# zhyever/PatchFusion

Hardware: AMD Instinct MI355X
Metric: patches/sec (DepthAnything-ViT-L PatchFusion, 4K image, P=16 tiles at N=1) (higher is better)
Workload: dtype f32; 1 GPU; Depth-Anything-vitl14 PatchFusion, 2160x3840 synthetic RGB, 4x4 regular tiling (cai_mode m1, 16 tiles), process_num=8, random-init weights (BASELINE.json configs[2] at N=1; 16 tiles per GPU); parallelism=single GPU

## Files before the change

include/pf_hip.h:

```cpp
#ifndef PF_HIP_H
#define PF_HIP_H
#include <stdint.h>

#ifdef __cplusplus
extern "C" {
#endif

#define PF_DTYPE_F32 0
#define PF_DTYPE_BF16 1

#define PF_ACT_NONE 0
#define PF_ACT_RELU 1
#define PF_ACT_GELU 2
#define PF_ACT_SOFTPLUS 3

const char* pf_last_error(void);
int pf_version(void);

typedef struct {
  const void* x; int x_ld; int B, H, W, Cin;
  const void* w; int w_rows; int Kpad;
  const float* bias; const float* scale;
  const void* res; int res_ld; const void* res2; int res2_ld;
  void* y; int y_ld; int OH, OW, Cout;
  int KH, KW, stride, pad;
  int act;
  int relu_in;
  int out_f32;
  int shuffle;
  int dtype;
  int korder;
  int batch;
  long x_bstride, w_bstride, y_bstride;
  const int* col_exp;
  const int* out_exp;
} pf_conv_params;
int pf_conv(const pf_conv_params* p, void* stream);
int pf_conv_timed(const pf_conv_params* p, int iters, float* ms, void* stream);

int pf_conv_winograd(const pf_conv_params* p, int m, const void* U, int u_rows, int u_kpad, void* V, void* M, void* stream);
int pf_conv_winograd_split3(const pf_conv_params* p, const void* U3, int u_rows, int u_kpad, void* V3, void* M, void* stream);
int pf_conv_winograd_split3_windowed(const pf_conv_params* p, const void* U3, int u_rows, int u_kpad, void* V3, void* M, long window, void* stream);
long pf_wino_f16x2_scratch_bytes(int cin, int u_rows);
int pf_conv_winograd_f16x2_supported(const pf_conv_params* p, int u_rows, int u_kpad, long window);
int pf_conv_winograd_f16x2_windowed(const pf_conv_params* p, const void* U, int u_rows, int u_kpad, void* V2, void* M, void* scratch, long window,
                                    void* stream);
int pf_gemm_f16x2_points(const pf_conv_params* p, const int* col_exp, int grid_cap, void* stream);
int pf_gemm_f16x2(const pf_conv_params* p, void* stream);

int pf_conv_winograd_fused_supported(const pf_conv_params* p);
int pf_conv_winograd_fused(const pf_conv_params* p, const void* up, int nnb, int gs, void* stream);
int pf_conv_winograd_fused_timed(const pf_conv_params* p, const void* up, int nnb, int gs, int iters, float* ms, void* stream);

int pf_gemm_split3(const pf_conv_params* p, void* stream);
int pf_conv1x1_split3(const pf_conv_params* p, const void* w3, int w3_rows, void* stream);
int pf_gemm_split3_ex(const pf_conv_params* p, int grid_cap, void* stream);
#define PF_S3_ROUTE_TILE64 0
#define PF_S3_ROUTE_TILE128 1
#define PF_S3_ROUTE_PERSIST128 2
#define PF_S3_ROUTE_PERSIST192 3
int pf_gemm_split3_route(const pf_conv_params* p, int cus);
int pf_gemm_split3_timed(const pf_conv_params* p, int iters, float* ms, void* stream);
int pf_gemm_bf16_pp(const pf_conv_params* p, void* stream);
int pf_layernorm_split3(const float* x, int x_ld, void* y3, int y_ld, long plane, int kmajor, const float* g, const float* b, float eps,
                        long rows, int D, void* stream);
int pf_layernorm_f16x2(const float* x, int x_ld, void* y2, const int* in_exp, const float* g, const float* b, float eps, long rows, int D,
                       void* stream);
int pf_vit_attention_qkv_split3(const void* qkv, void* out3, long plane, int kmajor, int B, int S, int Hh, void* stream);
int pf_vit_attention_split3(const void* qkv3, long plane_in, void* out3, long plane_out, int kmajor, int B, int S, int Hh, void* stream);
int pf_vit_attention_split3_v2(const void* qkv3, long plane_in, void* out3, long plane_out, int kmajor, int B, int S, int Hh, int queries_per_wave,
                               int schedule, void* stream);
int pf_vit_attention_split3_rpb(const void* qkv3, long plane_in, void* out3, long plane_out, int kmajor, int B, int S, int Hh, const float* tab,
                                int th, int tw, int queries_per_wave, void* stream);
int pf_split3(const float* x, int x_ld, void* y, int y_ld, long plane, long rows, int cols, void* stream);

int pf_patch_im2col(const float* img, int B, int H, int W, void* out, int ld, int dtype, void* stream);
int pf_patch_im2col_norm(const float* img, int B, int H, int W, int patch, const float* mean3, const float* std3, float* out, int ld, void* stream);
int pf_readout_concat(const float* x, int x_ld, int B, int S, int D, float* y, int y_ld, void* stream);
int pf_assemble_tokens(const void* emb, void* tokens, const float* cls, const float* pos, int B, int S, int D, int dtype,
                       void* stream);
int pf_layernorm(const void* x, int x_ld, void* y, int y_ld, const float* g, const float* b, float eps,
                 int batches, int in_rows_per_batch, int in_row_offset, int out_rows_per_batch, int D,
                 int dtype, void* stream);
int pf_qkv_split(const void* qkv, int B, int S, int Hh, void* q, void* k, void* vt, int Sp, float scale,
                 int dtype, void* stream);
int pf_vit_attention(const void* q, const void* k, const void* vt, void* out, int B, int S, int Sp, int Hh,
                     int dtype, void* stream);
int pf_vit_attention_qkv(const void* qkv, void* out, int B, int S, int Hh, int dtype, void* stream);

int pf_swin_ln_partition(const void* x, int x_ld, void* xw, const float* g, const float* b, float eps,
                         int B, int H, int W, int C, int shift, int dtype, void* stream);
int pf_swin_window_attention(const void* qkv, void* out, const float* bias_table, int B, int Hp, int Wp,
                             int C, int heads, int shift, int dtype, void* stream);
int pf_swin_unpartition_add(const void* proj, const void* shortcut, int s_ld, void* y, int y_ld, int B, int H,
                            int W, int C, int shift, int dtype, void* stream);
int pf_add_rowwise(void* x, int x_ld, const float* pos, int B, int T, int C, int dtype, void* stream);

int pf_resize_bilinear(const void* x, int x_ld, int B, int H, int W, int C, void* y, int y_ld, int OH, int OW,
                       const void* add, int add_ld, int in_f32, int out_f32, int dtype, void* stream);
int pf_resize_concat(const void* const* xs, const int* lds, const int* Hs, const int* Ws, const int* Cs, int nsrc, int B,
                     void* y, int y_ld, int OH, int OW, int dtype, void* stream);
int pf_crop_resize_planar(const float* img, int C, int H, int W, const int* boxes, int P, float* out, int oh, int ow,
                          void* stream);
int pf_roi_align(const void* feat, int f_ld, int Bf, int H, int W, int C, const float* rois, int K, void* y,
                 int y_ld, int oh, int ow, float spatial_scale, int in_f32, int out_f32, int dtype, void* stream);
int pf_maxpool2(const void* x, int x_ld, int B, int H, int W, int C, void* y, int y_ld, int dtype, void* stream);
int pf_copy_channels(const void* x, int x_ld, void* y, int y_ld, long npix, int C, int in_f32, int out_f32,
                     int dtype, void* stream);
int pf_pack_fusion_input(const float* cdepth, const float* fdepth, const float* crops, void* y, int B, int h, int w,
                         int dtype, void* stream);
int pf_nhwc_to_nchw_f32(const void* x, int x_ld, float* y, int B, int H, int W, int C, int in_f32, int dtype, void* stream);

int pf_attractor(const float* A, int a_ld, int n_attr, int a_stride, float a_eps, int attractor_exp, int kind_sum,
                 const float* b_prev, int hp, int wp, float* out, int B, int h, int w, int n_bins, void* stream);
int pf_seed_bin_centers(const float* x, int x_ld, float* out, long npix, int n_bins, float min_depth, float max_depth, int bounded,
                        int normalize, void* stream);
int pf_bounded_bin_centers(const float* b, float* out, long npix, int n_bins, float min_depth, float max_depth, void* stream);
int pf_logbinom_depth(const float* pt, int pt_ld, const float* centers, int hc, int wc, float* depth, int B, int h,
                      int w, int n_bins, float min_temp, float max_temp, void* stream);
int pf_bins_tail(const float* clb, int clb_ld, int rel_off, const float* emb, int he, int we, const float* w0f, const float* b0,
                 const float* w2, const float* b2, const float* centers, int hc, int wc, float* depth, int B, int H, int W, int nq,
                 float min_temp, float max_temp, void* stream);

int pf_stitch_init(float* pred, float* count, int MH, int MW, const float* depth, const float* mask, const int* yx,
                   int P, int ph, int pw, void* stream);
int pf_stitch_finish_init(float* avg, const float* pred, const float* count, long n, void* stream);
int pf_stitch_update(float* avg, float* count, int MH, int MW, const float* depth, int dh, int dw, const float* mask,
                     int y0, int x0, int ph, int pw, void* stream);
int pf_resize_nearest_f32(const float* x, int H, int W, float* y, int OH, int OW, void* stream);
int pf_resize_bilinear_f32(const float* x, int H, int W, float* y, int OH, int OW, void* stream);


int pf_u8_bicubic_to_f32(const uint8_t* src, int H, int W, int reverse_channels, float* dst, int OH, int OW, void* stream);

int pf_percentile_workspace_bytes(void);
int pf_percentiles_f32(const float* x, long n, float invalid_val, int use_invalid, const uint8_t* invalid_mask, double q0, double q1,
                       float* out2, void* workspace, void* stream);

int pf_colorize_f32(const float* depth, long n, const float* vmin_vmax, const uint8_t* lut_rgba, int N, float invalid_val,
                    int use_invalid, const uint8_t* invalid_mask, uint32_t background_rgba, uint8_t* out_rgba, void* stream);

int pf_depth_to_u16(const float* depth, long n, float scale, uint16_t* out, void* stream);

int pf_depth_metrics(const float* gt, int H, int W, const float* pred, int ph, int pw, const float* edges,
                     const uint8_t* additional_mask, float min_depth, float max_depth, int crop_y0, int crop_y1, int crop_x0, int crop_x1,
                     double* out13, void* stream);

int pf_silog_loss(const float* pred, const float* target, long n, float min_depth, float max_depth, float beta, double* ws3,
                  float* loss, void* stream);

#ifdef __cplusplus
}
#endif
#endif
```

patchfusion_amd/_lib.py:

```python
import ctypes as C
import os

import torch

_HERE = os.path.dirname(os.path.abspath(__file__))
LIB_PATH = os.environ.get("PF_LIB_PATH") or os.path.join(_HERE, "libpf_hip.so")

vp, ci, cf, cl = C.c_void_p, C.c_int, C.c_float, C.c_long


class ConvParams(C.Structure):
    _fields_ = [
        ("x", vp), ("x_ld", ci), ("B", ci), ("H", ci), ("W", ci), ("Cin", ci),
        ("w", vp), ("w_rows", ci), ("Kpad", ci),
        ("bias", vp), ("scale", vp),
        ("res", vp), ("res_ld", ci), ("res2", vp), ("res2_ld", ci),
        ("y", vp), ("y_ld", ci), ("OH", ci), ("OW", ci), ("Cout", ci),
        ("KH", ci), ("KW", ci), ("stride", ci), ("pad", ci),
        ("act", ci), ("relu_in", ci), ("out_f32", ci), ("shuffle", ci), ("dtype", ci), ("korder", ci),
        ("batch", ci), ("x_bstride", C.c_long), ("w_bstride", C.c_long), ("y_bstride", C.c_long),
        ("col_exp", vp), ("out_exp", vp),
    ]


SIGNATURES = {
    "pf_conv": [C.POINTER(ConvParams), vp],
    "pf_conv_timed": [C.POINTER(ConvParams), ci, C.POINTER(cf), vp],
    "pf_patch_im2col": [vp, ci, ci, ci, vp, ci, ci, vp],
    "pf_assemble_tokens": [vp, vp, vp, vp, ci, ci, ci, ci, vp],
    "pf_layernorm": [vp, ci, vp, ci, vp, vp, cf, ci, ci, ci, ci, ci, ci, vp],
    "pf_qkv_split": [vp, ci, ci, ci, vp, vp, vp, ci, cf, ci, vp],
    "pf_vit_attention": [vp, vp, vp, vp, ci, ci, ci, ci, ci, vp],
    "pf_vit_attention_qkv": [vp, vp, ci, ci, ci, ci, vp],
    "pf_swin_ln_partition": [vp, ci, vp, vp, vp, cf, ci, ci, ci, ci, ci, ci, vp],
    "pf_swin_window_attention": [vp, vp, vp, ci, ci, ci, ci, ci, ci, ci, vp],
    "pf_swin_unpartition_add": [vp, vp, ci, vp, ci, ci, ci, ci, ci, ci, ci, vp],
    "pf_add_rowwise": [vp, ci, vp, ci, ci, ci, ci, vp],
    "pf_resize_bilinear": [vp, ci, ci, ci, ci, ci, vp, ci, ci, ci, vp, ci, ci, ci, ci, vp],
    "pf_resize_concat": [C.POINTER(vp), C.POINTER(ci), C.POINTER(ci), C.POINTER(ci), C.POINTER(ci), ci, ci, vp, ci, ci, ci, ci, vp],
    "pf_crop_resize_planar": [vp, ci, ci, ci, vp, ci, vp, ci, ci, vp],
    "pf_roi_align": [vp, ci, ci, ci, ci, ci, vp, ci, vp, ci, ci, ci, cf, ci, ci, ci, vp],
    "pf_maxpool2": [vp, ci, ci, ci, ci, ci, vp, ci, ci, vp],
    "pf_copy_channels": [vp, ci, vp, ci, cl, ci, ci, ci, ci, vp],
    "pf_pack_fusion_input": [vp, vp, vp, vp, ci, ci, ci, ci, vp],
    "pf_nhwc_to_nchw_f32": [vp, ci, vp, ci, ci, ci, ci, ci, ci, vp],
    "pf_conv_winograd": [C.POINTER(ConvParams), ci, vp, ci, ci, vp, vp, vp],
    "pf_conv_winograd_split3": [C.POINTER(ConvParams), vp, ci, ci, vp, vp, vp],
    "pf_conv_winograd_split3_windowed": [C.POINTER(ConvParams), vp, ci, ci, vp, vp, C.c_long, vp],
    "pf_conv_winograd_f16x2_windowed": [C.POINTER(ConvParams), vp, ci, ci, vp, vp, vp, C.c_long, vp],
    "pf_gemm_f16x2_points": [C.POINTER(ConvParams), vp, ci, vp],
    "pf_gemm_f16x2": [C.POINTER(ConvParams), vp],
    "pf_gemm_split3": [C.POINTER(ConvParams), vp],
    "pf_gemm_split3_ex": [C.POINTER(ConvParams), ci, vp],
    "pf_conv1x1_split3": [C.POINTER(ConvParams), vp, ci, vp],
    "pf_gemm_split3_timed": [C.POINTER(ConvParams), ci, C.POINTER(cf), vp],
    "pf_gemm_bf16_pp": [C.POINTER(ConvParams), vp],
    "pf_split3": [vp, ci, vp, ci, cl, cl, ci, vp],
    "pf_layernorm_split3": [vp, ci, vp, ci, cl, ci, vp, vp, cf, cl, ci, vp],
    "pf_layernorm_f16x2": [vp, ci, vp, vp, vp, vp, cf, cl, ci, vp],
    "pf_vit_attention_qkv_split3": [vp, vp, cl, ci, ci, ci, ci, vp],
    "pf_vit_attention_split3": [vp, cl, vp, cl, ci, ci, ci, ci, vp],
    "pf_vit_attention_split3_v2": [vp, cl, vp, cl, ci, ci, ci, ci, ci, ci, vp],
    "pf_vit_attention_split3_rpb": [vp, cl, vp, cl, ci, ci, ci, ci, vp, ci, ci, ci, vp],
    "pf_patch_im2col_norm": [vp, ci, ci, ci, ci, vp, vp, vp, ci, vp],
    "pf_readout_concat": [vp, ci, ci, ci, ci, vp, ci, vp],
    "pf_conv_winograd_fused": [C.POINTER(ConvParams), vp, ci, ci, vp],
    "pf_conv_winograd_fused_timed": [C.POINTER(ConvParams), vp, ci, ci, ci, C.POINTER(cf), vp],
    "pf_attractor": [vp, ci, ci, ci, cf, ci, ci, vp, ci, ci, vp, ci, ci, ci, ci, vp],
    "pf_seed_bin_centers": [vp, ci, vp, cl, ci, cf, cf, ci, ci, vp],
    "pf_bounded_bin_centers": [vp, vp, cl, ci, cf, cf, vp],
    "pf_logbinom_depth": [vp, ci, vp, ci, ci, vp, ci, ci, ci, ci, cf, cf, vp],
    "pf_bins_tail": [vp, ci, ci, vp, ci, ci, vp, vp, vp, vp, vp, ci, ci, vp, ci, ci, ci, ci, cf, cf, vp],
    "pf_stitch_init": [vp, vp, ci, ci, vp, vp, vp, ci, ci, ci, vp],
    "pf_stitch_finish_init": [vp, vp, vp, cl, vp],
    "pf_stitch_update": [vp, vp, ci, ci, vp, ci, ci, vp, ci, ci, ci, ci, vp],
    "pf_resize_nearest_f32": [vp, ci, ci, vp, ci, ci, vp],
    "pf_resize_bilinear_f32": [vp, ci, ci, vp, ci, ci, vp],
    "pf_u8_bicubic_to_f32": [vp, ci, ci, ci, vp, ci, ci, vp],
    "pf_percentiles_f32": [vp, cl, cf, ci, vp, C.c_double, C.c_double, vp, vp, vp],
    "pf_colorize_f32": [vp, cl, vp, vp, ci, cf, ci, vp, C.c_uint32, vp, vp],
    "pf_depth_to_u16": [vp, cl, cf, vp, vp],
    "pf_silog_loss": [vp, vp, cl, cf, cf, cf, vp, vp, vp],
    "pf_depth_metrics": [vp, ci, ci, vp, ci, ci, vp, vp, cf, cf, ci, ci, ci, ci, vp, vp],
}
NON_STATUS = ("pf_last_error", "pf_version", "pf_percentile_workspace_bytes", "pf_conv_winograd_fused_supported", "pf_gemm_split3_route",
              "pf_wino_f16x2_scratch_bytes", "pf_conv_winograd_f16x2_supported")

_lib = None


def load():
    global _lib
    if _lib is not None:
        return _lib
    if not os.path.exists(LIB_PATH):
        raise ImportError(
            f"{LIB_PATH} not found: the HIP extension is not built. Run `python __graft_entry__.py` "
            "(or `make -C patchfusion_amd/csrc`). There is no CPU fallback for the product path.")
    lib = C.CDLL(LIB_PATH)
    for name, args in SIGNATURES.items():
        fn = getattr(lib, name)
        fn.argtypes = args
        fn.restype = ci
    lib.pf_last_error.restype = C.c_char_p
    lib.pf_last_error.argtypes = []
    lib.pf_version.restype = ci
    lib.pf_version.argtypes = []
    lib.pf_percentile_workspace_bytes.restype = ci
    lib.pf_percentile_workspace_bytes.argtypes = []
    lib.pf_conv_winograd_fused_supported.restype = ci
    lib.pf_conv_winograd_fused_supported.argtypes = [C.POINTER(ConvParams)]
    lib.pf_gemm_split3_route.restype = ci
    lib.pf_gemm_split3_route.argtypes = [C.POINTER(ConvParams), ci]
    lib.pf_wino_f16x2_scratch_bytes.restype = C.c_long
    lib.pf_wino_f16x2_scratch_bytes.argtypes = [ci, ci]
    lib.pf_conv_winograd_f16x2_supported.restype = ci
    lib.pf_conv_winograd_f16x2_supported.argtypes = [C.POINTER(ConvParams), ci, ci, C.c_long]
    _lib = lib
    return lib


class PfError(RuntimeError):
    pass


def check(rc, what):
    if rc != 0:
        msg = load().pf_last_error()
        raise PfError(f"{what} failed (status {rc}): {msg.decode() if msg else ''}")
```

patchfusion_amd/csrc/attn_split3.hip:

```cpp
#include "pf_common.h"
#include "../../include/pf_hip.h"

#include <cstdlib>
#include <type_traits>

namespace {

typedef short v4s __attribute__((__vector_size__(4 * sizeof(short))));
typedef short v8s __attribute__((__vector_size__(8 * sizeof(short))));
typedef __attribute__((address_space(3))) v4s lds_v4s;

__device__ __forceinline__ unsigned lds_addr_of(const void* p) {
  return (unsigned)(size_t)(__attribute__((address_space(3))) const char*)p;
}
__device__ __forceinline__ void dma16(const void* sbase, unsigned voff, unsigned lds_dst) {
  unsigned keep;
  asm volatile("s_mov_b32 %0, m0\n\ts_mov_b32 m0, %3\n\ts_nop 4\n\tglobal_load_lds_dwordx4 %1, %2\n\ts_mov_b32 m0, %0"
               : "=&s"(keep)
               : "v"(voff), "s"(sbase), "s"(lds_dst)
               : "memory");
}
__device__ __forceinline__ void barrier_lds() { asm volatile("s_waitcnt lgkmcnt(0)\n\ts_barrier" ::: "memory"); }
__device__ __forceinline__ void barrier_all() { asm volatile("s_waitcnt vmcnt(0) lgkmcnt(0)\n\ts_barrier" ::: "memory"); }

__device__ __forceinline__ bf16x8 tr_pair(const char* p0, const char* p1) {
  const v4s a = __builtin_amdgcn_ds_read_tr16_b64_v4i16((lds_v4s*)p0);
  const v4s b = __builtin_amdgcn_ds_read_tr16_b64_v4i16((lds_v4s*)p1);
  return __builtin_bit_cast(bf16x8, __builtin_shufflevector(a, b, 0, 1, 2, 3, 4, 5, 6, 7));
}

constexpr int KS_BYTES = 3 * 64 * 128;

struct RpbArgs {
  const float* tab;
  int th, tw;
};

template <int QG, bool RPB>
__device__ __forceinline__ void attn_v2_body(const bf16_t* __restrict__ qkv3, long plane_in, bf16_t* __restrict__ out3, long plane_out, int S,
                                             int Hh, float qscale, long kmaj_rows, int n_qb, int dbg, RpbArgs rpb) {
#ifdef PF_ATTN_DBG
#define ADBG(bit) (dbg & (bit))
#else
#define ADBG(bit) 0
#endif
  extern __shared__ __attribute__((aligned(16))) char smem[];
  char* const Ks = smem;
  char* const Vs = smem + KS_BYTES;
  constexpr int QW = 16 * QG, QB = 4 * QW;
  const int tid = threadIdx.x, lane = tid & 63;
  const int wave = __builtin_amdgcn_readfirstlane(tid >> 6);
  const int r = lane & 15, g = lane >> 4;
  const int bid = xcd_remap((int)blockIdx.x, (int)gridDim.x);
  const int bh = bid / n_qb, qb = bid - bh * n_qb;
  const int b = bh / Hh, h = bh - b * Hh;
  const int q0 = qb * QB + wave * QW;
  const bool has_q = q0 < S;
  const int D = Hh * 64;
  const long rs = 3L * D;
  const bf16_t* base = qkv3 + (long)b * S * rs + h * 64;
  const int ntiles = (S + 63) / 64;

  const unsigned rs_b = (unsigned)(rs * 2);
  const unsigned krow_off = (unsigned)(lane >> 3) * rs_b + (unsigned)(((lane & 7) ^ (lane >> 3)) << 4);
  const unsigned vrow_off = (unsigned)(lane >> 3) * rs_b + (unsigned)(((lane & 7) ^ (((lane >> 4) & 3) << 1)) << 4);
  const unsigned ks_lds = lds_addr_of(Ks), vs_lds = lds_addr_of(Vs);
  auto issue = [&](int kt, int which, unsigned lds_dst) {
    const unsigned lane_off = (which == 1 ? krow_off : vrow_off) + (unsigned)(kt * 64) * rs_b;
    const char* sb = reinterpret_cast<const char*>(base + which * D);
    if (kt * 64 + 64 <= S) {
#pragma unroll
      for (int i = 0; i < 6; ++i) {
        const int p = wave * 6 + i;
        dma16(sb + (long)(p >> 3) * plane_in * 2, lane_off + (unsigned)((p & 7) * 8) * rs_b, lds_dst + p * 1024);
      }
    } else {
#pragma unroll
      for (int i = 0; i < 6; ++i) {
        const int p = wave * 6 + i;
        const int over = max(kt * 64 + (p & 7) * 8 + (lane >> 3) - (S - 1), 0);
        dma16(sb + (long)(p >> 3) * plane_in * 2, lane_off + (unsigned)((p & 7) * 8 - over) * rs_b, lds_dst + p * 1024);
      }
    }
  };

  const float* rtab = reinterpret_cast<const float*>(smem + 3 * KS_BYTES);
  int qbase[QG], cls_at = 0;
  float inv_tw = 0.f;
  if constexpr (RPB) {
    const int th = rpb.th, tw = rpb.tw, wq = 2 * tw - 1, ntab = (2 * th - 1) * wq + 3;
    const int y_lo = (max(qb * QB, 1) - 1) / tw, y_hi = (max(min(qb * QB + QB, S) - 1, 1) - 1) / tw;
    const int nsub = (y_hi - y_lo + th) * wq;
    const float* src = rpb.tab + (long)h * ntab;
    float* dst = reinterpret_cast<float*>(smem + 3 * KS_BYTES);
    for (int i = tid; i < nsub; i += 256) dst[i] = src[y_lo * wq + i];
    if (tid < 3) dst[nsub + tid] = src[ntab - 3 + tid];
    cls_at = nsub;
    inv_tw = 1.0f / (float)tw;
#pragma unroll
    for (int qg = 0; qg < QG; ++qg) {
      const int qi = min(q0 + 16 * qg + r, S - 1);
      const int pi = max(qi - 1, 0), yi = pi / tw, xi = pi - yi * tw;
      qbase[qg] = qi == 0 ? -1 : (yi - y_lo + th - 1) * wq + xi + tw - 1;
    }
  }

  issue(0, 1, ks_lds);
  issue(0, 2, vs_lds);

  uint4 qf[QG][3][2];
#pragma unroll
  for (int qg = 0; qg < QG; ++qg) {
    const int qi = min(q0 + 16 * qg + r, S - 1);
#pragma unroll
    for (int pl = 0; pl < 3; ++pl)
#pragma unroll
      for (int kh = 0; kh < 2; ++kh) qf[qg][pl][kh] = *reinterpret_cast<const uint4*>(base + pl * plane_in + (long)qi * rs + 32 * kh + 8 * g);
  }
  f32x4 o[QG][4];
  float m_run[QG], l_run[QG];
#pragma unroll
  for (int qg = 0; qg < QG; ++qg) {
    m_run[qg] = -INFINITY;
    l_run[qg] = 0.f;
#pragma unroll
    for (int fd = 0; fd < 4; ++fd) o[qg][fd] = f32x4{0.f, 0.f, 0.f, 0.f};
  }

  const char* kb0 = Ks + r * 128 + ((g ^ (r & 7)) << 4);
  const char* kb1 = Ks + r * 128 + (((4 + g) ^ (r & 7)) << 4);
  const int vrow = 4 * g + (r >> 2), vx = (vrow >> 1) & 3;
  const char* vb[4];
#pragma unroll
  for (int fd = 0; fd < 4; ++fd) vb[fd] = Vs + vrow * 128 + ((fd ^ vx) << 5) + ((r & 3) << 3);

  __builtin_amdgcn_s_waitcnt(0x0070);
  barrier_lds();

  auto tile = [&](int kt, auto last_c) {
    constexpr bool LAST = decltype(last_c)::value;
    const int rem = S - kt * 64;
    const int nkf = LAST ? (rem + 15) >> 4 : 4;
    const int nkk = LAST ? (rem + 31) >> 5 : 2;
    const int vstage = (kt & 1) * KS_BYTES;
    if (!LAST && !ADBG(1)) issue(kt + 1, 2, vs_lds + ((kt + 1) & 1) * KS_BYTES);
    f32x4 sacc[QG][4];
#pragma unroll
    for (int qg = 0; qg < QG; ++qg)
#pragma unroll
      for (int kf = 0; kf < 4; ++kf) sacc[qg][kf] = f32x4{0.f, 0.f, 0.f, 0.f};
    if (has_q && !ADBG(4)) {
#pragma unroll
      for (int kf = 0; kf < 4; ++kf) {
        if (LAST && kf >= nkf) break;
        uint4 kfr[3][2];
// ... 417 lines not shown
    auto group = [&](auto n_c) {
      constexpr int n = decltype(n_c)::value;
      if constexpr (NSLOT > 0) {
        if constexpr (n < 3) {
          load_group(std::integral_constant<int, n + 1>{});
          __builtin_amdgcn_sched_barrier(0);
        }
        slot(n_c, std::integral_constant<int, 0>{});
        slot(n_c, std::integral_constant<int, 1>{});
        slot(n_c, std::integral_constant<int, 2>{});
        slot(n_c, std::integral_constant<int, 3>{});
        slot(n_c, std::integral_constant<int, 4>{});
        slot(n_c, std::integral_constant<int, 5>{});
        slot(n_c, std::integral_constant<int, 6>{});
        slot(n_c, std::integral_constant<int, 7>{});
        slot(n_c, std::integral_constant<int, 8>{});
        slot(n_c, std::integral_constant<int, 9>{});
        slot(n_c, std::integral_constant<int, 10>{});
        slot(n_c, std::integral_constant<int, 11>{});
      }
    };
    group(std::integral_constant<int, 0>{});
    group(std::integral_constant<int, 1>{});
    group(std::integral_constant<int, 2>{});
    group(std::integral_constant<int, 3>{});
    if constexpr (NSLOT == 0 && SM) {
#pragma unroll
      for (int i = 0; i < 16; ++i) sm_exp1(i);
      l_run = l_run * a_pend + psum;
#pragma unroll
      for (int u = 0; u < 8; ++u) { sm_split_a(u); sm_split_b(u); }
    }
  };
  auto turn = [&](int j, int ks, int vs) {
    TL_MARK(8);
    asm volatile("s_waitcnt vmcnt(6) lgkmcnt(0)\n\ts_barrier" ::: "memory");
    TL_MARK(1);
    issue(j + 4, 1, kr_lds + ks);
    issue(j + 2, 2, vr_lds + vs);
    TL_MARK(2);
  };
  using T = std::true_type;
  using F = std::false_type;
  using P0 = std::integral_constant<int, 0>;
  using P1 = std::integral_constant<int, 1>;
  if (!ksplit) {
    step(T{}, F{}, F{}, F{}, P1{}, 0, 0, 0);
    turn(-1, 0, PB_BYTES);
    if (NB > 1) step(T{}, T{}, F{}, F{}, P0{}, PB_BYTES, 0, 0);
    else step(F{}, T{}, T{}, F{}, P0{}, 0, 0, S);
    turn(0, PB_BYTES, 2 * PB_BYTES);
    int ks = 2 * PB_BYTES, vs = 0;
    int j = 1;
    for (; j + 1 <= NB - 2; j += 2) {
      step(T{}, T{}, F{}, T{}, P1{}, ks, vs, 0);
      turn(j, ks, vs);
      ks = ks == 2 * PB_BYTES ? 0 : ks + PB_BYTES;
      vs = vs == 2 * PB_BYTES ? 0 : vs + PB_BYTES;
      step(T{}, T{}, F{}, T{}, P0{}, ks, vs, 0);
      turn(j + 1, ks, vs);
      ks = ks == 2 * PB_BYTES ? 0 : ks + PB_BYTES;
      vs = vs == 2 * PB_BYTES ? 0 : vs + PB_BYTES;
    }
    if (j <= NB - 2) {
      step(T{}, T{}, F{}, T{}, P1{}, ks, vs, 0);
      turn(j, ks, vs);
      ks = ks == 2 * PB_BYTES ? 0 : ks + PB_BYTES;
      vs = vs == 2 * PB_BYTES ? 0 : vs + PB_BYTES;
      ++j;
    }
    const int rem = S - (NB - 1) * 32;
    if (NB > 1) {
      if (j & 1) step(F{}, T{}, T{}, T{}, P1{}, ks, vs, rem);
      else step(F{}, T{}, T{}, T{}, P0{}, ks, vs, rem);
      vs = vs == 2 * PB_BYTES ? 0 : vs + PB_BYTES;
      ++j;
    }
    barrier_all();
    if (j & 1) step(F{}, F{}, F{}, T{}, P1{}, 0, vs, 0);
    else step(F{}, F{}, F{}, T{}, P0{}, 0, vs, 0);
  } else {
    const int remk = S - (NB - 1) * 32;
    int ksj = 0, vsj = PB_BYTES;
    for (int jj = -1; jj <= NB; ++jj) {
      if (((jj + 1 - wave) & 3) == 0 && jj + 1 < NB) step(T{}, F{}, F{}, F{}, P1{}, ksj, vsj, 0);
      else if (((jj - wave) & 3) == 0 && jj >= 0 && jj < NB) {
        if (jj == NB - 1) step(F{}, T{}, T{}, F{}, P0{}, ksj, vsj, remk);
        else step(F{}, T{}, F{}, F{}, P0{}, ksj, vsj, 0);
      } else if (((jj - 1 - wave) & 3) == 0 && jj >= 1 && jj - 1 < NB) step(F{}, F{}, F{}, T{}, P1{}, ksj, vsj, 0);
      if (jj <= NB - 2) turn(jj, ksj, vsj);
      else if (jj == NB - 1) barrier_all();
      ksj = ksj == 2 * PB_BYTES ? 0 : ksj + PB_BYTES;
      vsj = vsj == 2 * PB_BYTES ? 0 : vsj + PB_BYTES;
    }
    __syncthreads();
    float* park = reinterpret_cast<float*>(smem);
    if (wave > 0) {
      float* pw = park + (wave - 1) * 34 * 64 + lane;
      pw[0] = m_run;
      pw[64] = l_run;
#pragma unroll
      for (int t = 0; t < 2; ++t)
#pragma unroll
        for (int i = 0; i < 16; ++i) pw[(2 + t * 16 + i) * 64] = o[t][i];
    }
    __syncthreads();
    if (wave > 0) return;
#pragma unroll 1
    for (int w = 0; w < 3; ++w) {
      const float* pw = park + w * 34 * 64 + lane;
      const float mw = pw[0], lw = pw[64];
      const float mn = fmaxf(m_run, mw);
      const float f0 = __builtin_amdgcn_exp2f(m_run - mn), fw = __builtin_amdgcn_exp2f(mw - mn);
      l_run = l_run * f0 + lw * fw;
#pragma unroll
      for (int t = 0; t < 2; ++t)
#pragma unroll
        for (int i = 0; i < 16; ++i) o[t][i] = o[t][i] * f0 + pw[(2 + t * 16 + i) * 64] * fw;
      m_run = mn;
    }
  }

  TL_MARK(10);
  if (!has_q) return;
  float l = l_run;
  {
    const auto y = __builtin_amdgcn_permlane32_swap(__float_as_uint(l), __float_as_uint(l), false, false);
    l = __uint_as_float(y[0]) + __uint_as_float(y[1]);
  }
  const float inv = 1.0f / l;
  const int qo = q0 + c;
  if (qo < S) {
#pragma unroll
    for (int t = 0; t < 2; ++t)
#pragma unroll
      for (int rq = 0; rq < 4; ++rq) {
        const int col = h * 64 + 32 * t + 8 * rq + 4 * hi;
        const float w4[4] = {o[t][4 * rq] * inv, o[t][4 * rq + 1] * inv, o[t][4 * rq + 2] * inv, o[t][4 * rq + 3] * inv};
        store_split3(out3 + split3_at((long)b * S + qo, col, D, kmaj_rows), plane_out, w4);
      }
  }
  TL_MARK(11);
  TL_FLUSH();
#ifdef PF_ATTN_DBG
  if (tid == 0 && blockIdx.x < 4096) {
    g_attn_blk[blockIdx.x][0] = blk_t0;
    g_attn_blk[blockIdx.x][1] = __builtin_amdgcn_s_memrealtime();
    g_attn_blk[blockIdx.x][2] = __builtin_amdgcn_s_getreg((31 << 11) | 4)   ;
    g_attn_blk[blockIdx.x][3] = __builtin_amdgcn_s_getreg((31 << 11) | 20)   ;
  }
#endif
}

constexpr int V2_LDS = 3 * KS_BYTES;

}

extern "C" int pf_vit_attention_split3_v2(const void* qkv3, long plane_in, void* out3, long plane_out, int kmajor, int B, int S, int Hh,
                                          int queries_per_wave, int schedule, void* stream) {
  if (!qkv3 || !out3 || B <= 0 || S <= 0 || Hh <= 0 || plane_in < (long)B * S * Hh * 192 || plane_out < (long)B * S * Hh * 64) return PF_ERR_ARG;
  if ((long)S * Hh * 192 * 2 >= (1L << 31)) return PF_ERR_ARG;
  if (queries_per_wave != 0 && queries_per_wave != 16 && queries_per_wave != 32) return PF_ERR_ARG;
  if (schedule < 0 || schedule > 2) return PF_ERR_ARG;
  const float qscale = 0.125f * 1.4426950408889634f;
  int dbg = 0, lds2 = V2_LDS, ldsp = PIPE_LDS;
#ifdef PF_ATTN_DBG
  if (const char* e = getenv("PF_ATTN_DBG")) dbg = atoi(e);
  if (const char* e = getenv("PF_ATTN_LDS")) lds2 = ldsp = atoi(e);
#endif
  static int attr_done = 0;
  if (attr_done != lds2) {
    const void* ks[3] = {reinterpret_cast<const void*>(vit_attention_split3_v2_kernel<1>), reinterpret_cast<const void*>(vit_attention_split3_v2_kernel<2>),
                         reinterpret_cast<const void*>(vit_attention_split3_pipe_kernel)};
    for (int i = 0; i < 3; ++i)
      if (hipFuncSetAttribute(ks[i], hipFuncAttributeMaxDynamicSharedMemorySize, i < 2 ? lds2 : ldsp) != hipSuccess) return PF_ERR_LAUNCH;
    attr_done = lds2;
  }
  int qw = queries_per_wave;
  if (schedule != 1) qw = 32;
  if (qw == 0) qw = (long)((S + 127) / 128) * B * Hh >= 512 ? 32 : 16;
  const int n_qb = (S + 4 * qw - 1) / (4 * qw);
  const long kmaj_rows = kmajor ? (long)B * S : 0L;
  hipStream_t st = reinterpret_cast<hipStream_t>(stream);
  const dim3 grid(n_qb * B * Hh), block(256);
#define ATTN_LAUNCH(KERNEL, LDS)                                                                                                          \
  hipLaunchKernelGGL(KERNEL, grid, block, LDS, st, (const bf16_t*)qkv3, plane_in, (bf16_t*)out3, plane_out, S, Hh, qscale, kmaj_rows, n_qb, dbg)
  if (schedule == 1) {
    if (qw == 32) ATTN_LAUNCH(vit_attention_split3_v2_kernel<2>, lds2);
    else ATTN_LAUNCH(vit_attention_split3_v2_kernel<1>, lds2);
  } else {
    hipLaunchKernelGGL(vit_attention_split3_pipe_kernel, grid, block, ldsp, st, (const bf16_t*)qkv3, plane_in, (bf16_t*)out3, plane_out, S, Hh, qscale, kmaj_rows, n_qb,
                       B * Hh, dbg);
  }
#undef ATTN_LAUNCH
  return hipGetLastError() == hipSuccess ? PF_OK : PF_ERR_LAUNCH;
}

extern "C" int pf_vit_attention_split3_rpb(const void* qkv3, long plane_in, void* out3, long plane_out, int kmajor, int B, int S, int Hh,
                                           const float* tab, int th, int tw, int queries_per_wave, void* stream) {
  if (!qkv3 || !out3 || !tab || B <= 0 || Hh <= 0 || th <= 0 || tw <= 0 || plane_in < (long)B * S * Hh * 192 || plane_out < (long)B * S * Hh * 64)
    return PF_ERR_ARG;
  if ((long)th * tw + 1 != S || S >= (1 << 20)) return PF_ERR_ARG;
  if ((long)S * Hh * 192 * 2 >= (1L << 31)) return PF_ERR_ARG;
  if (queries_per_wave != 0 && queries_per_wave != 16 && queries_per_wave != 32) return PF_ERR_ARG;
  int qw = queries_per_wave;
  if (qw == 0) qw = (long)((S + 127) / 128) * B * Hh >= 512 ? 32 : 16;
  const int QB = 4 * qw, n_qb = (S + QB - 1) / QB, wq = 2 * tw - 1;
  int rows = 0;
  for (int qb = 0; qb < n_qb; ++qb) {
    const int y_lo = ((qb * QB > 1 ? qb * QB : 1) - 1) / tw, last = (qb * QB + QB < S ? qb * QB + QB : S) - 1;
    const int y_hi = ((last > 1 ? last : 1) - 1) / tw;
    rows = rows > y_hi - y_lo + th ? rows : y_hi - y_lo + th;
  }
  const int lds = 3 * KS_BYTES + ((rows * wq + 3) * 4 + 15) / 16 * 16;
  if (lds > 160 * 1024) return PF_ERR_ARG;
  const void* k = qw == 32 ? reinterpret_cast<const void*>(vit_attention_split3_rpb_kernel<2>) : reinterpret_cast<const void*>(vit_attention_split3_rpb_kernel<1>);
  static int attr_lds[2] = {0, 0};
  if (attr_lds[qw == 32] < lds) {
    if (hipFuncSetAttribute(k, hipFuncAttributeMaxDynamicSharedMemorySize, lds) != hipSuccess) return PF_ERR_LAUNCH;
    attr_lds[qw == 32] = lds;
  }
  const float qscale = 0.125f * 1.4426950408889634f;
  const long kmaj_rows = kmajor ? (long)B * S : 0L;
  hipStream_t st = reinterpret_cast<hipStream_t>(stream);
  const dim3 grid(n_qb * B * Hh), block(256);
  if (qw == 32)
    hipLaunchKernelGGL(vit_attention_split3_rpb_kernel<2>, grid, block, lds, st, (const bf16_t*)qkv3, plane_in, (bf16_t*)out3, plane_out, S, Hh, qscale, kmaj_rows,
                       n_qb, tab, th, tw);
  else
    hipLaunchKernelGGL(vit_attention_split3_rpb_kernel<1>, grid, block, lds, st, (const bf16_t*)qkv3, plane_in, (bf16_t*)out3, plane_out, S, Hh, qscale, kmaj_rows,
                       n_qb, tab, th, tw);
  return hipGetLastError() == hipSuccess ? PF_OK : PF_ERR_LAUNCH;
}

#ifdef PF_ATTN_DBG
extern "C" int pf_attn_dbg_blocks(long long* out, int nblocks) {
  hipDeviceSynchronize();
  return hipMemcpyFromSymbol(out, HIP_SYMBOL(g_attn_blk), sizeof(long long) * 4 * (nblocks < 4096 ? nblocks : 4096)) == hipSuccess ? PF_OK : PF_ERR_LAUNCH;
}
extern "C" int pf_attn_dbg_timeline(long long* out48) {
  hipDeviceSynchronize();
  return hipMemcpyFromSymbol(out48, HIP_SYMBOL(g_attn_tl), sizeof(long long) * 48) == hipSuccess ? PF_OK : PF_ERR_LAUNCH;
}
#endif
```

patchfusion_amd/csrc/gemm_split3.hip:

```cpp
#include <atomic>
#include <type_traits>
#include "pf_common.h"
#include "../../include/pf_hip.h"

namespace {

__device__ __attribute__((aligned(256))) unsigned int s3_zero_page[64];

__device__ __forceinline__ unsigned lds_addr(const void* p) {
  return (unsigned)(size_t)(__attribute__((address_space(3))) const char*)p;
}
__device__ __forceinline__ void glds16(const void* gsrc, unsigned lds_dst) {
  unsigned keep;
  asm volatile("s_mov_b32 %0, m0\n\ts_mov_b32 m0, %2\n\ts_nop 0\n\tglobal_load_lds_dwordx4 %1, off\n\ts_mov_b32 m0, %0"
               : "=&s"(keep)
               : "v"(gsrc), "s"(lds_dst)
               : "memory");
}

template <int N>
__device__ __forceinline__ void vm_wait() { asm volatile("s_waitcnt vmcnt(%0)" ::"n"(N) : "memory"); }
__device__ __forceinline__ void lds_barrier() { asm volatile("s_waitcnt lgkmcnt(0)\n\ts_barrier" ::: "memory"); }

__device__ __forceinline__ void plain_barrier() {
// ... 516 lines not shown
  auto decode = [&](int l, int& z, int& m0, int& n0) __attribute__((always_inline)) {
    z = l / per_plane;
    const int r = l - z * per_plane;
    if (gm == 0) {
      const int t = r / nt;
      m0 = t * BM;
      n0 = (r - t * nt) * BN;
      return;
    }
    const int group = r / per_group, in_g = r - group * per_group, first = group * gm;
    const int gsz = min(mt - first, gm);
    const int tn = in_g / gsz;
    m0 = (first + in_g - tn * gsz) * BM;
    n0 = tn * BN;
  };

  const bool is_x = wave < WM;
  const bool kmaj = (p.korder & (is_x ? 2 : 4)) != 0;
  const int lim = is_x ? M : p.w_rows;
  const int ld_b = kmaj ? 64 : (is_x ? p.x_ld : p.Kpad) * 2;
  const unsigned adv_b = kmaj ? (unsigned)lim * 64u : 64u;
  const unsigned long long op_base = is_x ? (unsigned long long)p.x : (unsigned long long)p.w;
  const unsigned long long pl_b = (unsigned long long)(is_x ? p.x_bstride : p.w_bstride) * 2;
  const unsigned long long z_b = (unsigned long long)lim * ((is_x ? p.x_ld : p.Kpad) * 2);
  unsigned long long sbase[PPW];
  unsigned voff[PPW];
  auto setup_loader = [&](int l) __attribute__((always_inline)) {
    int z, m0, n0;
    decode(l, z, m0, n0);
#ifdef PF_S3_DBG
    if (p.pad & 16) { m0 = 0; if (is_x) z = 0; }
#endif
    const int origin = is_x ? m0 : n0;
    const unsigned long long tb = op_base + (unsigned long long)z * z_b + (unsigned long long)origin * ld_b;
    const int last = lim - 1 - origin;

    int lane_o = lane;
    asm volatile("" : "+v"(lane_o));
#pragma unroll
    for (int i = 0; i < PPW; ++i) {
      const int pc = (wave & (WM - 1)) * PPW + i;
      const int row = pc * 16 + (lane_o >> 2);
      const int j = (lane_o & 3) ^ ((row >> 1) & 3);
      const int pl = pc / (BM / 16), r = row - pl * BM;
      sbase[i] = tb + pl * pl_b;
      voff[i] = (unsigned)(min(r, last) * ld_b + j * 16);
    }
  };
  const unsigned smem_base = lds_addr(smem);
  int l_load = l_first, l_kc = -1, s_issue = NS - 1;
  unsigned dst_cur = 0;
  setup_loader(l_load);
  auto begin_issue = [&]() __attribute__((always_inline)) {
    if constexpr (NS == 2) s_issue ^= 1;
    else s_issue = s_issue + 1 == NS ? 0 : s_issue + 1;
    if (++l_kc == nk) {
      l_kc = 0;
      l_load += nb;
      if (l_load < hi) setup_loader(l_load);
    }
    dst_cur = __builtin_amdgcn_readfirstlane(smem_base + s_issue * STAGE + wave * (PPW * 1024));
  };
  auto piece = [&](int i) __attribute__((always_inline)) {
    glds16s(voff[i], sbase[i], dst_cur + i * 1024);
    sbase[i] += adv_b;
  };
  auto issue = [&]() __attribute__((always_inline)) {
    begin_issue();
#pragma unroll
    for (int i = 0; i < PPW; ++i) piece(i);
  };

  f32x4 acc[FN][FM];
#pragma unroll
  for (int fn = 0; fn < FN; ++fn)
#pragma unroll
    for (int fm = 0; fm < FM; ++fm) acc[fn][fm] = f32x4{0.f, 0.f, 0.f, 0.f};

  const int fr = lane & 15, fg = lane >> 4;
  const int slot = (fg ^ ((fr >> 1) & 3)) << 4;
  const int x_off = (wm * WTM + fr) * 64 + slot;
  constexpr int NFN_MIN = 3;
  int cur_nfn = FN, cur_wtn = WTN, e_nfn = FN, e_wtn = WTN;
  int w_off = NP * BM * 64 + (wn * WTN + fr) * 64 + slot;
  auto tile_shape = [&](int n0) __attribute__((always_inline)) {
    if (!(flags & 8)) return;
    const int nv = min(BN, p.Cout - n0);
    cur_nfn = min(FN, max(NFN_MIN, ((nv + 15) / 16 + WN - 1) / WN));
    cur_wtn = cur_nfn * 16;
    w_off = NP * BM * 64 + (wn * cur_wtn + fr) * 64 + slot;
  };
  struct Frags { uint4 w[NP][FN], x[NP][FM]; };
  Frags f;
  int s_read = 0;
  auto read_frags = [&]() __attribute__((always_inline)) {
    const char* S = smem + s_read * STAGE;
    if constexpr (NS == 2) s_read ^= 1;
    else s_read = s_read + 1 == NS ? 0 : s_read + 1;
#pragma unroll
    for (int pl = 0; pl < NP; ++pl) {
#pragma unroll
      for (int fn = 0; fn < FN; ++fn)
        if (fn < NFN_MIN || fn < cur_nfn) f.w[pl][fn] = *reinterpret_cast<const uint4*>(S + w_off + pl * (BN * 64) + fn * 1024);
#pragma unroll
      for (int fm = 0; fm < FM; ++fm) f.x[pl][fm] = *reinterpret_cast<const uint4*>(S + x_off + pl * (BM * 64) + fm * 1024);
    }
  };
#define S3_TERM192(TI, PW, PX)                                                                                                  \
  _Pragma("unroll") for (int fn = 0; fn < FN; ++fn) _Pragma("unroll") for (int fm = 0; fm < FM; ++fm) {                      \
    if (ISS && ((TI) * FN * FM + fn * FM + fm) % MPP == 0) {                                                                   \
      __builtin_amdgcn_sched_barrier(0);                                                                                       \
      piece(((TI) * FN * FM + fn * FM + fm) / MPP);                                                                            \
      __builtin_amdgcn_sched_barrier(0);                                                                                       \
    }                                                                                                                          \
    if (fn < NFN_MIN || fn < cur_nfn) {                                                                                        \
      if constexpr (F16)                                                                                                       \
        acc[fn][fm] = __builtin_amdgcn_mfma_f32_16x16x32_f16(__builtin_bit_cast(f16x8, f.w[PW][fn]), __builtin_bit_cast(f16x8, f.x[PX][fm]), \
                                                             acc[fn][fm], 0, 0, 0);                                            \
      else                                                                                                                     \
        acc[fn][fm] = __builtin_amdgcn_mfma_f32_16x16x32_bf16(__builtin_bit_cast(bf16x8, f.w[PW][fn]), __builtin_bit_cast(bf16x8, f.x[PX][fm]), \
                                                              acc[fn][fm], 0, 0, 0);                                           \
    }                                                                                                                          \
  }
  auto multiply = [&](auto with_issue) __attribute__((always_inline)) {
    constexpr bool ISS = decltype(with_issue)::value;
    if constexpr (F16) {
      S3_TERM192(0, 0, 1) S3_TERM192(1, 1, 0) S3_TERM192(2, 0, 0)
    } else {
      S3_TERM192(0, 0, 2) S3_TERM192(1, 2, 0) S3_TERM192(2, 1, 1) S3_TERM192(3, 0, 1) S3_TERM192(4, 1, 0) S3_TERM192(5, 0, 0)
    }
  };
#undef S3_TERM192

  int l_comp = l_first, c_kc = 0;
  int e_z = 0, e_m0 = 0, e_n0 = 0;
  bool epi_pending = false;
  auto epilogue = [&]() __attribute__((always_inline)) {
    const long y_base = (long)e_z * M * p.y_ld;
    int fr = lane & 15, fg = lane >> 4;
    asm volatile("" : "+v"(fr), "+v"(fg));
    const bool lo = fr < 8, oddg = fg & 1;
#pragma unroll
    for (int fn = 0; fn < FN; fn += 2) {
      __builtin_amdgcn_sched_barrier(0);
      const int fsel = fn + (lo ? 0 : 1);
      const int n = e_n0 + wn * e_wtn + fsel * 16 + fg * 4;
      const bool nok = n < p.Cout && fsel < e_nfn;
      float4 bias_r = make_float4(0.f, 0.f, 0.f, 0.f), scale_r = make_float4(1.f, 1.f, 1.f, 1.f);
      int4 fexp = make_int4(0, 0, 0, 0), oexp = make_int4(0, 0, 0, 0);
      if constexpr (F16 && BARE) {
        if (nok) fexp = *reinterpret_cast<const int4*>(reinterpret_cast<const int*>(p.scale) + (long)e_z * p.w_rows + n);
      } else if constexpr (F16) {
        if (nok) fexp = *reinterpret_cast<const int4*>(p.col_exp + n);
        if (nok && (p.korder & 16)) oexp = *reinterpret_cast<const int4*>(p.out_exp + n);
      }
      if constexpr (!BARE) {
        if (nok) {
          if (p.bias) bias_r = *reinterpret_cast<const float4*>(p.bias + n);
          if (p.scale) scale_r = *reinterpret_cast<const float4*>(p.scale + n);
        }
      }
#pragma unroll
      for (int fm = 0; fm < FM; ++fm) {
        const f32x4 a = acc[fn][fm], b = acc[fn + 1][fm];
        acc[fn][fm] = f32x4{0.f, 0.f, 0.f, 0.f};
        acc[fn + 1][fm] = f32x4{0.f, 0.f, 0.f, 0.f};
        float v[2][4];
#pragma unroll
        for (int r = 0; r < 4; ++r) {
          const float snd = lo ? b[r] : a[r];
          const float recv = __builtin_bit_cast(float, __builtin_amdgcn_update_dpp(0, __builtin_bit_cast(int, snd), 0x128, 0xf, 0xf, false));
          v[0][r] = lo ? a[r] : recv;
          v[1][r] = lo ? recv : b[r];
        }
        const int m1 = e_m0 + wm * WTM + fm * 16 + (fr & 7);
        if constexpr (F16) {
          const int fe[4] = {fexp.x, fexp.y, fexp.z, fexp.w};
#pragma unroll
          for (int r = 0; r < 4; ++r) { v[0][r] = ldexpf(v[0][r], fe[r]); v[1][r] = ldexpf(v[1][r], fe[r]); }
        }
        if constexpr (BARE) {
          float* yb = reinterpret_cast<float*>(p.y) + y_base;
          if (nok && m1 < M) *reinterpret_cast<float4*>(yb + (long)m1 * p.y_ld + n) = make_float4(v[0][0], v[0][1], v[0][2], v[0][3]);
          if (nok && m1 + 8 < M) *reinterpret_cast<float4*>(yb + (long)(m1 + 8) * p.y_ld + n) = make_float4(v[1][0], v[1][1], v[1][2], v[1][3]);
        } else {
          const float bs[4] = {bias_r.x, bias_r.y, bias_r.z, bias_r.w}, sc[4] = {scale_r.x, scale_r.y, scale_r.z, scale_r.w};
          const int ne = n - (oddg ? 4 : 0);
          uint32_t lw[2][2];
#pragma unroll
          for (int h = 0; h < 2; ++h) {
            __builtin_amdgcn_sched_barrier(0);
            const int m = m1 + 8 * h;
            const bool ok = nok && m < M;
#pragma unroll
            for (int r = 0; r < 4; ++r) v[h][r] += bs[r];
            if (p.act == PF_ACT_RELU) {
#pragma unroll
              for (int r = 0; r < 4; ++r) v[h][r] = fmaxf(v[h][r], 0.f);
            } else if (p.act == PF_ACT_GELU) {
#pragma unroll
              for (int r = 0; r < 4; ++r) v[h][r] = gelu_erf(v[h][r]);
            } else if (p.act == PF_ACT_SOFTPLUS) {
#pragma unroll
              for (int r = 0; r < 4; ++r) v[h][r] = softplus20(v[h][r]);
            }
#pragma unroll
            for (int r = 0; r < 4; ++r) v[h][r] *= sc[r];
            if (p.res && ok) {
              const float4 q = *reinterpret_cast<const float4*>(reinterpret_cast<const float*>(p.res) + (long)m * p.res_ld + n);
              v[h][0] += q.x; v[h][1] += q.y; v[h][2] += q.z; v[h][3] += q.w;
            }
            if (p.res2 && ok) {
              const float4 q = *reinterpret_cast<const float4*>(reinterpret_cast<const float*>(p.res2) + (long)m * p.res2_ld + n);
              v[h][0] += q.x; v[h][1] += q.y; v[h][2] += q.z; v[h][3] += q.w;
            }
            if (p.out_f32) {
              if (ok) *reinterpret_cast<float4*>(reinterpret_cast<float*>(p.y) + y_base + (long)m * p.y_ld + n) = make_float4(v[h][0], v[h][1], v[h][2], v[h][3]);
            } else if (F16 && (p.korder & 16)) {
              const int oe[4] = {oexp.x, oexp.y, oexp.z, oexp.w};
              uint32_t hw[2], lw2[2];
#pragma unroll
              for (int r = 0; r < 4; r += 2) {
                const float t0 = ldexpf(v[h][r], -oe[r]), t1 = ldexpf(v[h][r + 1], -oe[r + 1]);
                const _Float16 h0 = (_Float16)t0, h1 = (_Float16)t1;
                const _Float16 l0 = (_Float16)(t0 - (float)h0), l1 = (_Float16)(t1 - (float)h1);
                hw[r >> 1] = (uint32_t)__builtin_bit_cast(uint16_t, h0) | ((uint32_t)__builtin_bit_cast(uint16_t, h1) << 16);
                lw2[r >> 1] = (uint32_t)__builtin_bit_cast(uint16_t, l0) | ((uint32_t)__builtin_bit_cast(uint16_t, l1) << 16);
              }
              const auto s0 = __builtin_amdgcn_permlane16_swap(hw[0], lw2[0], false, false);
              const auto s1 = __builtin_amdgcn_permlane16_swap(hw[1], lw2[1], false, false);
              if (ok) *reinterpret_cast<uint4*>(reinterpret_cast<uint16_t*>(p.y) + split3_at(m, ne, p.y_ld, M) + (oddg ? p.y_bstride : 0)) = make_uint4(s0[0], s1[0], s0[1], s1[1]);
            } else if (F16 || !(p.korder & 8)) {
              if (ok) store_split3(reinterpret_cast<bf16_t*>(p.y) + split3_at(m, n, p.y_ld, 0), p.y_bstride, v[h]);
            } else {
              uint32_t h0, m0, h1, mm1;
              split3_pair(v[h][0], v[h][1], h0, m0, lw[h][0]);
              split3_pair(v[h][2], v[h][3], h1, mm1, lw[h][1]);
              const auto s0 = __builtin_amdgcn_permlane16_swap(h0, m0, false, false);
              const auto s1 = __builtin_amdgcn_permlane16_swap(h1, mm1, false, false);
              if (ok) *reinterpret_cast<uint4*>(reinterpret_cast<bf16_t*>(p.y) + split3_at(m, ne, p.y_ld, M) + (oddg ? p.y_bstride : 0)) = make_uint4(s0[0], s1[0], s0[1], s1[1]);
            }
          }
          if (!F16 && !p.out_f32 && (p.korder & 8)) {
            const auto t0 = __builtin_amdgcn_permlane16_swap(lw[0][0], lw[1][0], false, false);
            const auto t1 = __builtin_amdgcn_permlane16_swap(lw[0][1], lw[1][1], false, false);
            const int ml = m1 + (oddg ? 8 : 0);
            if (nok && ml < M) *reinterpret_cast<uint4*>(reinterpret_cast<bf16_t*>(p.y) + split3_at(ml, ne, p.y_ld, M) + 2 * p.y_bstride) = make_uint4(t0[0], t1[0], t0[1], t1[1]);
          }
        }
      }
    }
    epi_pending = false;
  };
  auto tile_cursor = [&]() __attribute__((always_inline)) {
    if (epi_pending) epilogue();
    if (c_kc == 0) {
      int z, m0, n0;
      decode(l_comp, z, m0, n0);
      tile_shape(n0);
    }
    if (c_kc == nk - 1) {
      decode(l_comp, e_z, e_m0, e_n0);
      e_nfn = cur_nfn;
      e_wtn = cur_wtn;
      l_comp += nb;
    }
  };
  auto tile_advance = [&]() __attribute__((always_inline)) {
    if (++c_kc == nk) { c_kc = 0; epi_pending = true; }
  };

#ifdef PF_S3_DBG
  unsigned long long* tl = nullptr;
  if constexpr (BARE) tl = reinterpret_cast<unsigned long long*>(const_cast<void*>(p.res2));
  const bool stamp_w = tl && blockIdx.x == 0 && (wave == 0 || wave == 4);
#define S3_STAMP192(g, k)                                                                                     \
  if (stamp_w && (g) >= 64 && (g) < 96) {                                                                     \
    __builtin_amdgcn_sched_barrier(0);                                                                        \
    const unsigned long long t_ = __builtin_amdgcn_s_memtime();                                               \
    if (lane == 0) tl[(((wave >> 2) * 32 + ((g) - 64)) << 3) + (k)] = t_;                                      \
    __builtin_amdgcn_sched_barrier(0);                                                                        \
  }
#else
#define S3_STAMP192(g, k)
#endif
  issue();
  if (LEAD == 2 && chunks > 1) {
    issue();
    vm_wait<PPW>();
  } else {
    vm_wait<0>();
  }
  lds_barrier();
  auto wait_next = [&](int g) __attribute__((always_inline)) {
    if (LEAD == 2 && g + 2 < chunks) vm_wait<PPW>();
    else vm_wait<0>();
  };
  if (wave < NW / 2) {
#pragma nounroll
    for (int g = 0; g < chunks; ++g) {
      S3_STAMP192(g, 0)
      tile_cursor();
      S3_STAMP192(g, 1)
      if (g + LEAD < chunks) issue();
      S3_STAMP192(g, 2)
      read_frags();
      S3_STAMP192(g, 3)
      lds_barrier();
      S3_STAMP192(g, 4)
      __builtin_amdgcn_sched_barrier(0);
      __builtin_amdgcn_s_setprio(1);
      multiply(std::false_type{});
      __builtin_amdgcn_s_setprio(0);
      S3_STAMP192(g, 5)
      tile_advance();
      wait_next(g);
      S3_STAMP192(g, 6)
      plain_barrier();
      S3_STAMP192(g, 7)
    }
    plain_barrier();
  } else if constexpr (BL) {
    plain_barrier();
#pragma nounroll
    for (int g = 0; g < chunks; ++g) {
      S3_STAMP192(g, 0)
      tile_cursor();
      S3_STAMP192(g, 1)
      if (g + LEAD < chunks) issue();
      S3_STAMP192(g, 2)
      read_frags();
      S3_STAMP192(g, 3)
      wait_next(g);
      S3_STAMP192(g, 4)
      lds_barrier();
      S3_STAMP192(g, 5)
      __builtin_amdgcn_sched_barrier(0);
      __builtin_amdgcn_s_setprio(1);
      multiply(std::false_type{});
      __builtin_amdgcn_s_setprio(0);
      S3_STAMP192(g, 6)
      tile_advance();
      plain_barrier();
      S3_STAMP192(g, 7)
    }
  } else {
    if (1 < chunks) issue();
    plain_barrier();
    int g = 0;
#pragma nounroll
    for (; g + 2 < chunks; ++g) {
      tile_cursor();
      begin_issue();
      read_frags();
      vm_wait<0>();
      lds_barrier();
      __builtin_amdgcn_sched_barrier(0);
      __builtin_amdgcn_s_setprio(1);
      multiply(std::true_type{});
      __builtin_amdgcn_s_setprio(0);
      tile_advance();
      plain_barrier();
    }
#pragma nounroll
    for (; g < chunks; ++g) {
      tile_cursor();
      read_frags();
      vm_wait<0>();
      lds_barrier();
      __builtin_amdgcn_sched_barrier(0);
      __builtin_amdgcn_s_setprio(1);
      multiply(std::false_type{});
      __builtin_amdgcn_s_setprio(0);
      tile_advance();
      plain_barrier();
    }
  }
  epilogue();
}

thread_local char g_err[200] = {0};
constexpr int PF_ERR_FALLBACK = -100;

int cu_count() {
// ... 98 lines not shown
    hipFuncSetAttribute(reinterpret_cast<const void*>(gemm_split3_persist192_kernel<true, true, true, 3>), hipFuncAttributeMaxDynamicSharedMemorySize, 3 * stage);
    hipFuncSetAttribute(reinterpret_cast<const void*>(gemm_split3_persist192_kernel<true, true, true, 2>), hipFuncAttributeMaxDynamicSharedMemorySize, 2 * stage);
    done.fetch_or(bit, std::memory_order_release);
  }
  const char* sl = getenv("PF_F16_SLOTS");
  const bool three = !(sl && sl[0] == '2');
  const long M = (long)p.B * p.OH * p.OW;
  const int mt = (int)((M + 191) / 192), nt = (p.Cout + 191) / 192;
  const long total = (long)mt * nt * (p.batch > 1 ? p.batch : 1);
  const int gm = tile_group(nt);
  int grid = cu_count();
  if (grid_cap > 0 && grid_cap < grid) grid = grid_cap;
  if (grid > total) grid = (int)total;
  grid &= ~7;
  if (total > 0x7fffffffL || grid < 8) return PF_ERR_ARG;
  if (three) hipLaunchKernelGGL((gemm_split3_persist192_kernel<true, true, true, 3>), dim3((unsigned)grid), dim3(512), 3 * stage, st, p, mt, nt, gm, (int)total, 8);
  else hipLaunchKernelGGL((gemm_split3_persist192_kernel<true, true, true, 2>), dim3((unsigned)grid), dim3(512), 2 * stage, st, p, mt, nt, gm, (int)total, 8);
  return hipGetLastError() == hipSuccess ? PF_OK : PF_ERR_LAUNCH;
}

int launch_persist192_f16_linear(const pf_conv_params& p, hipStream_t st) {
  constexpr int smem = 3 * 2 * (192 + 192) * 64;
  static std::atomic<unsigned long long> done{0};
  int dev = 0;
  hipGetDevice(&dev);
  const unsigned long long bit = 1ull << (dev & 63);
  if (!(done.load(std::memory_order_acquire) & bit)) {
    hipFuncSetAttribute(reinterpret_cast<const void*>(gemm_split3_persist192_kernel<false, true, true, 3>), hipFuncAttributeMaxDynamicSharedMemorySize, smem);
    done.fetch_or(bit, std::memory_order_release);
  }
  const long M = (long)p.B * p.OH * p.OW;
  const int mt = (int)((M + 191) / 192), nt = (p.Cout + 191) / 192;
  const long total = (long)mt * nt;
  const int gm = tile_group(nt);
  int grid = cu_count();
  if (grid > total) grid = (int)total;
  grid &= ~7;
  if (grid < 8) grid = 8;
  if (total > 0x7fffffffL) return PF_ERR_ARG;
  hipLaunchKernelGGL((gemm_split3_persist192_kernel<false, true, true, 3>), dim3((unsigned)grid), dim3(512), smem, st, p, mt, nt, gm, (int)total, 8);
  return hipGetLastError() == hipSuccess ? PF_OK : PF_ERR_LAUNCH;
}

template <int BM, int BN, int WM, int WN, int NS, bool PP = false, int NP = 3, bool PLAIN = false>
int launch(const pf_conv_params& p, hipStream_t st) {
  constexpr int smem = NS * NP * (BM + BN) * 64;
  static std::atomic<unsigned long long> done{0};
  int dev = 0;
  hipGetDevice(&dev);
  const unsigned long long bit = 1ull << (dev & 63);
  auto kern = gemm_split3_kernel<BM, BN, WM, WN, NS, PP, NP, PLAIN>;
  if (!(done.load(std::memory_order_acquire) & bit)) {
    hipFuncSetAttribute(reinterpret_cast<const void*>(kern), hipFuncAttributeMaxDynamicSharedMemorySize, smem);
    done.fetch_or(bit, std::memory_order_release);
  }
  const long M = (long)p.B * p.OH * p.OW;
  const long tiles = ((M + BM - 1) / BM) * ((p.Cout + BN - 1) / BN);
  hipLaunchKernelGGL(kern, dim3((unsigned)tiles, (unsigned)(p.batch > 1 ? p.batch : 1)), dim3(64 * WM * WN), smem, st, p);
  return hipGetLastError() == hipSuccess ? PF_OK : PF_ERR_LAUNCH;
}

int split3_route(const pf_conv_params& p, int cus) {
  int force = 0;
  if (const char* s = getenv("PF_S3_TILE_NOW")) force = atoi(s);
  const long M = (long)p.B * p.OH * p.OW;
  const long t128 = ((M + 127) / 128) * ((p.Cout + 127) / 128);
  const long planes = p.batch > 1 ? p.batch : 1;
  if (force ? force == 64 : t128 * planes < cus) return PF_S3_ROUTE_TILE64;
  const char* ps = getenv("PF_S3_PERSIST");
  if (!(ps && ps[0] == '0') && p.Cin >= 96 && (t128 * planes >= 2L * cus || (ps && ps[0] == '2')) && t128 * planes >= 8) {
    const char* ts = getenv("PF_S3_T192");
    const long t192 = ((M + 191) / 192) * ((p.Cout + 191) / 192);
    const long cost128 = ((t128 * planes + cus - 1) / cus) * 100, cost192 = ((t192 * planes + cus - 1) / cus) * 210 + 50;
    const bool want = ts && ts[0] == '2' ? true : (ts && ts[0] == '0' ? false : cost192 < cost128);
    return want && t192 * planes >= 8 ? PF_S3_ROUTE_PERSIST192 : PF_S3_ROUTE_PERSIST128;
  }
  return PF_S3_ROUTE_TILE128;
}

}

extern "C" int pf_gemm_split3_route(const pf_conv_params* p, int cus) {
  if (!p || cus <= 0) return -1;
  return split3_route(*p, cus);
}

namespace {
}

extern "C" int pf_gemm_split3(const pf_conv_params* p, void* stream) { return pf_gemm_split3_ex(p, 0, stream); }

extern "C" int pf_gemm_split3_ex(const pf_conv_params* p, int grid_cap, void* stream) {
  const char* e = nullptr;
  if (!p || !p->x || !p->w || !p->y) return PF_ERR_ARG;
#ifdef PF_S3_DBG
  pf_conv_params pd = *p;
  if (const char* s = getenv("PF_S3_DBG")) pd.pad = atoi(s);
  p = &pd;
  if (p->KH != 1 || p->KW != 1 || p->stride != 1 || p->shuffle > 1) e = "1x1 / linear layers only";
#else
  if (p->KH != 1 || p->KW != 1 || p->stride != 1 || p->pad != 0 || p->shuffle > 1) e = "1x1 / linear layers only";
#endif
  else if (p->Cin <= 0 || p->Cin % 32 || p->Kpad < p->Cin || p->Kpad % 32 || p->x_ld % 8 || p->x_ld < p->Cin) e = "K must be a multiple of 32, x_ld of 8";
  else if (p->Cout <= 0 || p->Cout % 4 || p->y_ld % 4 || p->w_rows < p->Cout) e = "Cout / y_ld must be multiples of 4";
  else if ((p->res && p->res_ld % 4) || (p->res2 && p->res2_ld % 4)) e = "residual ld must be a multiple of 4";
  else if ((long)p->B * p->OH * p->OW <= 0 || (long)p->B * p->OH * p->OW >= (1L << 31)) e = "bad token count";
  else if (p->x_bstride <= 0 || p->w_bstride <= 0 || (!p->out_f32 && p->y_bstride <= 0)) e = "plane strides missing";
  else if (((p->korder & 2) && p->x_ld != p->Cin) || ((p->korder & 4) && p->Kpad != p->Cin) || (p->korder & ~14)) e = "chunk-major operands are dense: x_ld == Kpad == Cin";
  else if ((p->korder & 8) && (p->out_f32 || p->y_ld != p->Cout || p->Cout % 32)) e = "chunk-major output: three planes, y_ld == Cout, Cout % 32 == 0";
  else if (((p->korder & 2) && (long)p->B * p->OH * p->OW * 64 >= (1L << 31)) || ((p->korder & 4) && (long)p->w_rows * 64 >= (1L << 31)))
    e = "too many rows for a chunk-major slab";
#ifdef PF_S3_DBG
  else if (p->batch > 1 && (!p->out_f32 || p->bias || p->scale || p->res || p->batch > 65535)) e = "batched planes: float32 output, no epilogue";
#else
  else if (p->batch > 1 && (!p->out_f32 || p->bias || p->scale || p->res || p->res2 || p->batch > 65535)) e = "batched planes: float32 output, no epilogue";
#endif
  if (e) return PF_ERR_ARG;
  hipStream_t st = reinterpret_cast<hipStream_t>(stream);
  switch (split3_route(*p, cu_count())) {
    case PF_S3_ROUTE_TILE64: return launch<64, 128, 2, 2, 2>(*p, st);
    case PF_S3_ROUTE_PERSIST192: {
      const int rc = launch_persist192(*p, st, grid_cap);
      if (rc != PF_ERR_FALLBACK) return rc;
      break;
    }
    case PF_S3_ROUTE_PERSIST128: {
      const int rc = launch_persist(*p, st, grid_cap);
      if (rc != PF_ERR_FALLBACK) return rc;
      break;
    }
    default: break;
  }
  const char* pp = getenv("PF_S3_PP");
  return (pp && pp[0] == '0') ? launch<128, 128, 4, 2, 3, false>(*p, st) : launch<128, 128, 4, 2, 3, true>(*p, st);
}

extern "C" int pf_gemm_f16x2_points(const pf_conv_params* p, const int* col_exp, int grid_cap, void* stream) {
  if (!p || !p->x || !p->w || !p->y || !col_exp) return PF_ERR_ARG;
  const long M = (long)p->B * p->OH * p->OW;
  if (p->KH != 1 || p->KW != 1 || p->stride != 1 || p->pad != 0 || p->shuffle > 1 || p->korder != 6 || !p->out_f32) return PF_ERR_ARG;
  if (p->Cin <= 0 || p->Cin % 32 || p->x_ld != p->Cin || p->Kpad != p->Cin || p->Cout <= 0 || p->Cout % 4 || p->y_ld % 4 || p->w_rows < p->Cout ||
      p->w_rows % 4)
    return PF_ERR_ARG;
  if (M <= 0 || M * 64 >= (1L << 31) || (long)p->w_rows * 64 >= (1L << 31) || p->x_bstride <= 0 || p->w_bstride <= 0) return PF_ERR_ARG;
  if (p->bias || p->scale || p->res || p->res2 || p->act != PF_ACT_NONE || p->batch > 65535) return PF_ERR_ARG;
  pf_conv_params q = *p;
  q.scale = reinterpret_cast<const float*>(col_exp);
  return launch_persist192_f16(q, reinterpret_cast<hipStream_t>(stream), grid_cap);
}

extern "C" int pf_gemm_f16x2(const pf_conv_params* p, void* stream) {
  if (!p || !p->x || !p->w || !p->y || !p->col_exp) return PF_ERR_ARG;
  const long M = (long)p->B * p->OH * p->OW;
  if (p->KH != 1 || p->KW != 1 || p->stride != 1 || p->pad != 0 || p->shuffle > 1 || p->batch > 1 || (p->korder & ~16) != 6) return PF_ERR_ARG;
  if (p->Cin <= 0 || p->Cin % 32 || p->x_ld != p->Cin || p->Kpad != p->Cin || p->Cout <= 0 || p->Cout % 4 || p->y_ld % 4 || p->w_rows < p->Cout ||
      p->w_rows % 4)
    return PF_ERR_ARG;
  if (M <= 0 || M * 64 >= (1L << 31) || (long)p->w_rows * 64 >= (1L << 31) || p->x_bstride <= 0 || p->w_bstride <= 0) return PF_ERR_ARG;
  if ((p->res && p->res_ld % 4) || (p->res2 && p->res2_ld % 4)) return PF_ERR_ARG;
  if (p->out_f32 && (p->korder & 16)) return PF_ERR_ARG;
  if (!p->out_f32 && p->y_bstride <= 0) return PF_ERR_ARG;
  if ((p->korder & 16) && (!p->out_exp || p->y_ld != p->Cout || p->Cout % 32)) return PF_ERR_ARG;
  return launch_persist192_f16_linear(*p, reinterpret_cast<hipStream_t>(stream));
}

extern "C" int pf_gemm_bf16_pp(const pf_conv_params* p, void* stream) {
  if (!p || !p->x || !p->w || !p->y) return PF_ERR_ARG;
  if (p->KH != 1 || p->KW != 1 || p->stride != 1 || p->pad != 0 || p->shuffle > 1 || p->dtype != PF_DTYPE_BF16) return PF_ERR_ARG;
  if (p->Cin <= 0 || p->Cin % 64 || p->Kpad < p->Cin || p->x_ld % 8 || p->x_ld < p->Cin || p->Kpad % 8) return PF_ERR_ARG;
  if (p->Cout <= 0 || p->Cout % 4 || p->y_ld % 4 || p->w_rows < p->Cout || (p->res && p->res_ld % 4) || (p->res2 && p->res2_ld % 4)) return PF_ERR_ARG;
  if ((long)p->B * p->OH * p->OW <= 0 || (long)p->B * p->OH * p->OW >= (1L << 31)) return PF_ERR_ARG;
  pf_conv_params pd = *p;
  pd.korder = 0;
  pd.x_bstride = 32;
  pd.w_bstride = 32;
  return launch<256, 128, 4, 2, 3, true, 2, true>(pd, reinterpret_cast<hipStream_t>(stream));
}

extern "C" int pf_gemm_split3_timed(const pf_conv_params* p, int iters, float* ms, void* stream) {
  if (!ms || iters <= 0) return PF_ERR_ARG;
  hipStream_t st = reinterpret_cast<hipStream_t>(stream);
  int rc = pf_gemm_split3(p, stream);
  if (rc != PF_OK) return rc;
  hipEvent_t e0, e1;
  hipEventCreate(&e0);
  hipEventCreate(&e1);
  hipEventRecord(e0, st);
  for (int i = 0; i < iters && rc == PF_OK; ++i) rc = pf_gemm_split3(p, stream);
  hipEventRecord(e1, st);
  hipEventSynchronize(e1);
  float t = 0.f;
  hipEventElapsedTime(&t, e0, e1);
  *ms = t / iters;
  hipEventDestroy(e0);
  hipEventDestroy(e1);
  return rc;
}

__global__ void split3_kernel(const float* __restrict__ x, int x_ld, bf16_t* __restrict__ y, int y_ld, long plane, long rows, int cols) {
  const int cv = cols >> 2;
  for (long i = (long)blockIdx.x * blockDim.x + threadIdx.x; i < rows * cv; i += (long)gridDim.x * blockDim.x) {
    const long r = i / cv;
    const int c = (int)(i - r * cv) * 4;
    const float4 a = *reinterpret_cast<const float4*>(x + r * x_ld + c);
    const float v[4] = {a.x, a.y, a.z, a.w};
    store_split3(y + r * y_ld + c, plane, v);
  }
}

extern "C" int pf_split3(const float* x, int x_ld, void* y, int y_ld, long plane, long rows, int cols, void* stream) {
  if (!x || !y || cols % 4 || x_ld % 4 || y_ld % 4 || rows <= 0 || plane <= 0) return PF_ERR_ARG;
  long n = rows * (cols / 4);
  long g = (n + 255) / 256;
  hipLaunchKernelGGL(split3_kernel, dim3((unsigned)(g > 16384 ? 16384 : g)), dim3(256), 0, reinterpret_cast<hipStream_t>(stream), x, x_ld,
                     static_cast<bf16_t*>(y), y_ld, plane, rows, cols);
  return hipGetLastError() == hipSuccess ? PF_OK : PF_ERR_LAUNCH;
}
```

patchfusion_amd/engine.py:

```python
import math

import torch

from . import packing as pk
from .config import pyramid_sizes
from .spec import DPT_ARCH, VIT_ARCH, branch_channels

F32 = torch.float32


def linear_split3_enabled():
    import os
    return os.environ.get("PF_LINEAR_SPLIT3", "1") != "0"


def vit_f16x2_enabled(crops):
    import os
    v = os.environ.get("PF_VIT_F16X2", "1")
    return v == "2" or (v != "0" and crops)


def attention_split3_enabled():
    import os
    return os.environ.get("PF_ATTN_SPLIT3", "1") != "0"


def bins_tail_enabled():
    import os
    return os.environ.get("PF_BINS_TAIL", "1") != "0"


def _g(sd, name, device):
    return sd[name].detach().to(device=device, dtype=F32).contiguous()


class BinsHead:

    def __init__(self, sd, prefix, C, bcfg, dtype, device, with_rel, min_depth=None, max_depth=None):
        self.dtype, self.device = dtype, device
        kind = bcfg.get("bin_centers_type", "softplus")
        if kind not in ("normed", "softplus", "hybrid1", "hybrid2"):
            raise ValueError("bin_centers_type should be one of 'normed', 'softplus', 'hybrid1', 'hybrid2'")
        self.seed_bounded, self.attr_bounded = kind in ("normed", "hybrid1"), kind in ("normed", "hybrid2")
        self.lo = float(bcfg.get("min_depth", 1e-3) if min_depth is None else min_depth)
        self.hi = float(bcfg.get("max_depth", 10) if max_depth is None else max_depth)
        if not with_rel and not ("attractor_type" in bcfg and "attractor_kind" in bcfg):
            raise AttributeError("coarse_branch config needs attractor_type and attractor_kind for the fusion head (patchfusion.py:162)")
        self.attr_type, self.attr_kind = bcfg.get("attractor_type", "exp"), bcfg.get("attractor_kind", "sum")
        if self.attr_kind not in ("mean", "sum"):
            raise KeyError(self.attr_kind)
        self.n_attr = list(bcfg["n_attractors"])
        self.n_bins = int(bcfg["n_bins"])
        self.emb = int(bcfg["bin_embedding_dim"])
        self.min_temp, self.max_temp = float(bcfg["min_temp"]), float(bcfg["max_temp"])
        self.with_rel = with_rel

        def pc(name, **kw):
            return pk.pack_conv(sd[prefix + name + ".weight"], sd[prefix + name + ".bias"], dtype=dtype, **kw).to(device)

        self.sbr0, self.sbr2 = pc("seed_bin_regressor._net.0"), pc("seed_bin_regressor._net.2")
        self.sp0, self.sp2 = pc("seed_projector._net.0"), pc("seed_projector._net.2")
        self.proj = [(pc(f"projectors.{i}._net.0"), pc(f"projectors.{i}._net.2")) for i in range(4)]
        self.attr = [(pc(f"attractors.{i}._net.0"), pc(f"attractors.{i}._net.2")) for i in range(4)]
        if with_rel:
            cmap, ctot = [(0, 32, 0), (32, 1, 32 + self.emb), (33, self.emb, 32)], 32 + self.emb + 8
        else:
            cmap, ctot = [(0, 32, 0), (33, self.emb, 32)], 32 + self.emb
        self.clb_channels = ctot
        self.mlp0 = pc("conditional_log_binomial.mlp.0", cin_map=cmap, cin_total=ctot)
        self.mlp2 = pc("conditional_log_binomial.mlp.2")
        self.tail = None
        if dtype == F32 and self.n_bins == 64 and bins_tail_enabled():
            self.tail = pk.bins_tail_weights(self.mlp0, self.mlp2, self.emb)
            if self.tail is not None:
                self.tail = self.tail.to(device)

    def new_clb_buffer(self, ops, B, H, W):
        return ops.empty((B, H, W, self.clb_channels), self.dtype, self.device)

    def run(self, ops, x0, x_blocks, clb, taps=None):
        dt, dev = self.dtype, self.device
        B, h0, w0, _ = x0.shape
        t = ops.empty((B, h0, w0, self.sbr0.cout), dt, dev)
        ops.conv(x0, self.sbr0, t, act="relu")
        b_prev = ops.empty((B, h0, w0, self.n_bins), F32, dev)
        ops.conv(t, self.sbr2, b_prev, act="relu" if self.seed_bounded else "softplus")
        if self.seed_bounded or self.attr_bounded:
            b_prev = ops.seed_bin_centers(b_prev, ops.empty((B, h0, w0, self.n_bins), F32, dev), self.lo, self.hi,
                                          bounded=self.seed_bounded, normalize=self.attr_bounded)
        t = ops.empty((B, h0, w0, self.sp0.cout), dt, dev)
        ops.conv(x0, self.sp0, t, act="relu")
        prev_emb = ops.empty((B, h0, w0, self.emb), dt, dev)
        ops.conv(t, self.sp2, prev_emb)
        emb = prev_emb
        for i, xb in enumerate(x_blocks):
            _, h, w, _ = xb.shape
            p0, p2 = self.proj[i]
            t = ops.empty((B, h, w, p0.cout), dt, dev)
            ops.conv(xb, p0, t, act="relu")
            emb = ops.empty((B, h, w, self.emb), dt, dev)
            ops.conv(t, p2, emb)
            xs = ops.empty((B, h, w, self.emb), dt, dev)
            ops.resize(prev_emb, xs, add=emb)
            a0, a2 = self.attr[i]
            t = ops.empty((B, h, w, a0.cout), dt, dev)
            ops.conv(xs, a0, t, act="relu")
            A = ops.empty((B, h, w, a2.cout), F32, dev)
            ops.conv(t, a2, A, act="relu" if self.attr_bounded else "softplus")
            b_new = ops.empty((B, h, w, self.n_bins), F32, dev)
            if self.attr_bounded:
                ops.attractor(A, self.n_attr[i], b_prev, b_new, a_stride=2, a_eps=1e-3, attractor_type=self.attr_type, kind=self.attr_kind)
            else:
                ops.attractor(A, self.n_attr[i], b_prev, b_new, attractor_type=self.attr_type, kind=self.attr_kind)
            b_prev, prev_emb = b_new, emb
            if taps is not None:
                taps[f"bins_centers{i}"] = b_new
        _, H, W, _ = clb.shape
        if self.tail is not None and emb.is_contiguous():
            if self.attr_bounded:
                b_prev = ops.bounded_bin_centers(b_prev, ops.empty(tuple(b_prev.shape), F32, dev), self.lo, self.hi)
            depth = ops.empty((B, H, W), F32, dev)
            ops.bins_tail(clb, emb, self.tail, b_prev, depth, self.min_temp, self.max_temp)
            return depth
        ops.resize(emb, clb[..., 32:32 + self.emb])
        t = ops.empty((B, H, W, self.mlp0.cout), dt, dev)
        ops.conv(clb, self.mlp0, t, act="gelu")
        pt = ops.empty((B, H, W, self.mlp2.cout), F32, dev)
        ops.conv(t, self.mlp2, pt, act="softplus")
        depth = ops.empty((B, H, W), F32, dev)
        if self.attr_bounded:
            b_prev = ops.bounded_bin_centers(b_prev, ops.empty(tuple(b_prev.shape), F32, dev), self.lo, self.hi)
        ops.logbinom_depth(pt, b_prev, depth, self.min_temp, self.max_temp)
        return depth


class BranchNet:

    def __init__(self, sd, prefix, bcfg, process_shape, dtype, device, ops=None, crops=False):
        self.dtype, self.device = dtype, device
        enc = bcfg["midas_model_type"]
        self.D, self.depth, self.heads = VIT_ARCH[enc]
        self.C, self.oc = DPT_ARCH[enc]
        self.H, self.W = process_shape
        self.th, self.tw = self.H // 14, self.W // 14
        v = prefix + "core.core.pretrained."
        h = prefix + "core.core.depth_head."
        dev = device

        def pc(name, bias=True, **kw):
            return pk.pack_conv(sd[name + ".weight"], sd[name + ".bias"] if bias else None, dtype=dtype, **kw).to(dev)

        w = sd[v + "patch_embed.proj.weight"]
        self.pe = pk.pack_conv(w.permute(0, 2, 3, 1).reshape(w.shape[0], -1), sd[v + "patch_embed.proj.bias"], dtype=dtype,
                               cin_total=592).to(dev)
        self.pos = pk.vit_pos_embed(sd[v + "pos_embed"], self.th, self.tw).to(dev)
        self.cls = _g(sd, v + "cls_token", dev).reshape(-1)
        self.split3 = dtype == F32 and linear_split3_enabled()
        if self.split3:
            def pc(name, bias=True, _pc=pc, **kw):
                if ".blocks." in name:
                    return pk.pack_conv_split3(sd[name + ".weight"], sd[name + ".bias"] if bias else None, **kw).to(dev)
                return _pc(name, bias, **kw)
        self.f16x2 = self.split3 and vit_f16x2_enabled(crops) and getattr(ops, "conv_f16x2", None) is not None
        self.blocks = []
        for i in range(self.depth):
            b = f"{v}blocks.{i}."
            n1, n2 = (sd[b + "norm1.weight"], sd[b + "norm1.bias"]), (sd[b + "norm2.weight"], sd[b + "norm2.bias"])
            if self.f16x2:
                bn1, bn2 = pk.layernorm_bound(*n1), pk.layernorm_bound(*n2)
                w1, b1 = sd[b + "mlp.fc1.weight"], sd[b + "mlp.fc1.bias"]
                qkv = pk.pack_conv_f16x2(sd[b + "attn.qkv.weight"], sd[b + "attn.qkv.bias"], None, bn1).to(dev)
                fc1 = pk.pack_conv_f16x2(w1, b1, None, bn2).to(dev)
                fc2 = pk.pack_conv_f16x2(sd[b + "mlp.fc2.weight"], sd[b + "mlp.fc2.bias"], sd[b + "ls2.gamma"],
                                         pk.gelu_linear_bound(w1, b1, bn2)).to(dev)
            else:
                qkv, fc1, fc2 = pc(b + "attn.qkv"), pc(b + "mlp.fc1"), pc(b + "mlp.fc2", scale=sd[b + "ls2.gamma"])
            self.blocks.append(dict(
                n1=(_g(sd, b + "norm1.weight", dev), _g(sd, b + "norm1.bias", dev)),
                qkv=qkv,
                proj=pc(b + "attn.proj", scale=sd[b + "ls1.gamma"]),
                n2=(_g(sd, b + "norm2.weight", dev), _g(sd, b + "norm2.bias", dev)),
                fc1=fc1,
                fc2=fc2))
        self.norm = (_g(sd, v + "norm.weight", dev), _g(sd, v + "norm.bias", dev))
        self.projects = [pc(f"{h}projects.{i}") for i in range(4)]
        self.up4 = pk.pack_conv_transpose(sd[h + "resize_layers.0.weight"], sd[h + "resize_layers.0.bias"], dtype=dtype).to(dev)
        self.up2 = pk.pack_conv_transpose(sd[h + "resize_layers.1.weight"], sd[h + "resize_layers.1.bias"], dtype=dtype).to(dev)
        self.down2 = pc(h + "resize_layers.3")
        self.rn = [pc(f"{h}scratch.layer{i + 1}_rn", bias=False) for i in range(4)]
        self.refine = {}
        for i in range(1, 5):
            r = f"{h}scratch.refinenet{i}."
            self.refine[i] = dict(out=pc(r + "out_conv"),
                                  u1=(pc(r + "resConfUnit1.conv1"), pc(r + "resConfUnit1.conv2")),
                                  u2=(pc(r + "resConfUnit2.conv1"), pc(r + "resConfUnit2.conv2")))
        self.oc1 = pc(h + "scratch.output_conv1")
        self.oc2a = pc(h + "scratch.output_conv2.0")
        self.oc2b = pk.pack_conv(sd[h + "scratch.output_conv2.2.weight"], sd[h + "scratch.output_conv2.2.bias"], dtype=dtype).to(dev)
        self.oc2b.cout = 8
        self.conv2 = pc(prefix + "conv2")
        self.head = BinsHead(sd, prefix, self.C, bcfg, dtype, dev, with_rel=True)

    def _rcu(self, ops, x, unit, extra_res=None):
        c1, c2 = unit
        t = ops.empty(x.shape[:3] + (c1.cout,), self.dtype, self.device)
        ops.conv(x, c1, t, pad=1, act="relu", relu_in=True)
        y = ops.empty(x.shape[:3] + (c2.cout,), self.dtype, self.device)
        ops.conv(t, c2, y, pad=1, res=x, res2=extra_res)
        return y

    def _refine(self, ops, idx, x, skip, size):
        r = self.refine[idx]
        if skip is not None:
            x = self._rcu(ops, skip, r["u1"], extra_res=x)
        x = self._rcu(ops, x, r["u2"])
        B, _, _, Cc = x.shape
        u = ops.empty((B, size[0], size[1], Cc), self.dtype, self.device)
        ops.resize(x, u)
        y = ops.empty((B, size[0], size[1], r["out"].cout), self.dtype, self.device)
        ops.conv(u, r["out"], y)
        return y

    def vit(self, ops, img, taps=None):
        dt, dev = self.dtype, self.device
        B = img.shape[0]
        T, S, D = self.th * self.tw, self.th * self.tw + 1, self.D
        col = ops.empty((B * T, 592), dt, dev)
        ops.patch_im2col(img, col)
        emb = ops.empty((B * T, D), dt, dev)
        ops.conv(col, self.pe, emb)
        tok = ops.empty((B, S, D), dt, dev)
        ops.assemble_tokens(emb, tok, self.cls, self.pos)
        x = tok.view(B * S, D)
        if taps is not None:
            taps["vit_tokens_in"] = tok.clone()
        feats = []
        if self.split3:
            if pk.split3_kmajor_enabled():
                hbuf, att, mid = (ops.empty((3, n // 32, B * S, 32), torch.bfloat16, dev) for n in (D, D, 4 * D))
            else:
                hbuf, att, mid = (ops.empty((3, B * S, n), torch.bfloat16, dev) for n in (D, D, 4 * D))
            qkv = ops.empty((3, B * S, 3 * D), torch.bfloat16, dev) if attention_split3_enabled() else ops.empty((B * S, 3 * D), dt, dev)
            if self.f16x2:
                hbuf, mid = (ops.empty((2, n // 32, B * S, 32), torch.float16, dev) for n in (D, 4 * D))
        else:
            hbuf = ops.empty((B * S, D), dt, dev)
            qkv = ops.empty((B * S, 3 * D), dt, dev)
            att = ops.empty((B * S, D), dt, dev)
            mid = ops.empty((B * S, 4 * D), dt, dev)
        for i, blk in enumerate(self.blocks):
            if self.f16x2:
                ops.layernorm_f16x2(x, hbuf, blk["n1"][0], blk["n1"][1], 1e-6, blk["qkv"].in_exp)
                ops.conv_f16x2(hbuf, blk["qkv"], qkv)
                ops.vit_attention(qkv, att, B, S, self.heads)
                ops.conv_split3(att, blk["proj"], x, res=x)
                ops.layernorm_f16x2(x, hbuf, blk["n2"][0], blk["n2"][1], 1e-6, blk["fc1"].in_exp)
                ops.conv_f16x2(hbuf, blk["fc1"], mid, act="gelu", out_exp=blk["fc2"].in_exp)
                ops.conv_f16x2(mid, blk["fc2"], x, res=x)
            elif self.split3:
                ops.layernorm_split3(x, hbuf, blk["n1"][0], blk["n1"][1], 1e-6)
                ops.conv_split3(hbuf, blk["qkv"], qkv)
                ops.vit_attention(qkv, att, B, S, self.heads)
                ops.conv_split3(att, blk["proj"], x, res=x)
                ops.layernorm_split3(x, hbuf, blk["n2"][0], blk["n2"][1], 1e-6)
                ops.conv_split3(hbuf, blk["fc1"], mid, act="gelu")
                ops.conv_split3(mid, blk["fc2"], x, res=x)
            else:
                ops.layernorm(x, hbuf, blk["n1"][0], blk["n1"][1], 1e-6)
                ops.conv(hbuf, blk["qkv"], qkv)
                ops.vit_attention(qkv, att, B, S, self.heads)
                ops.conv(att, blk["proj"], x, res=x)
                ops.layernorm(x, hbuf, blk["n2"][0], blk["n2"][1], 1e-6)
                ops.conv(hbuf, blk["fc1"], mid, act="gelu")
                ops.conv(mid, blk["fc2"], x, res=x)
            if taps is not None and i in (0, self.depth - 1):
                taps[f"vit_block{i}"] = x.view(B, S, D).clone()
            if i >= self.depth - 4:
                f = ops.empty((B, self.th, self.tw, D), dt, dev)
                ops.layernorm(x, f.view(B * T, D), self.norm[0], self.norm[1], 1e-6, batches=B, in_rows_per_batch=S,
                              in_row_offset=1, out_rows_per_batch=T)
                feats.append(f)
        return feats

    def forward(self, ops, img, taps=None, vit_feats=None):
        dt, dev = self.dtype, self.device
        B = img.shape[0]
        th, tw, C = self.th, self.tw, self.C
        feats = self.vit(ops, img, taps) if vit_feats is None else vit_feats
        if taps is not None:
            for i, f in enumerate(feats):
                taps[f"vit_out{i}"] = f
        maps = []
        for i, f in enumerate(feats):
            p = ops.empty((B, th, tw, self.projects[i].cout), dt, dev)
            ops.conv(f, self.projects[i], p)
            if i == 0:
                y = ops.empty((B, th * 4, tw * 4, self.oc[0]), dt, dev)
                ops.conv(p, self.up4, y)
            elif i == 1:
                y = ops.empty((B, th * 2, tw * 2, self.oc[1]), dt, dev)
                ops.conv(p, self.up2, y)
            elif i == 2:
                y = p
            else:
                y = ops.empty((B, (th + 1) // 2, (tw + 1) // 2, self.oc[3]), dt, dev)
                ops.conv(p, self.down2, y, stride=2, pad=1)
            maps.append(y)
        rn = []
        for i in range(4):
            y = ops.empty(maps[i].shape[:3] + (C,), dt, dev)
            ops.conv(maps[i], self.rn[i], y, pad=1)
            rn.append(y)
        r4 = self._refine(ops, 4, rn[3], None, rn[2].shape[1:3])
        r3 = self._refine(ops, 3, r4, rn[2], rn[1].shape[1:3])
        r2 = self._refine(ops, 2, r3, rn[1], rn[0].shape[1:3])
        r1 = self._refine(ops, 1, r2, rn[0], (rn[0].shape[1] * 2, rn[0].shape[2] * 2))
        o1 = ops.empty(r1.shape[:3] + (self.oc1.cout,), dt, dev)
        ops.conv(r1, self.oc1, o1, pad=1)
        H, W = th * 14, tw * 14
        o1u = ops.empty((B, H, W, self.oc1.cout), dt, dev)
        ops.resize(o1, o1u)
        clb = self.head.new_clb_buffer(ops, B, H, W)
        out_conv = clb[..., 0:32]
        ops.conv(o1u, self.oc2a, out_conv, pad=1, act="relu")
        ops.conv(out_conv, self.oc2b, clb[..., 32 + self.head.emb:], act="relu")
        x_d0 = ops.empty(rn[3].shape[:3] + (C,), dt, dev)
        ops.conv(rn[3], self.conv2, x_d0)
        if taps is not None:
            taps.update(dpt_layer1_rn=rn[0], dpt_layer4_rn=rn[3], rel_depth=clb[..., 32 + self.head.emb:33 + self.head.emb])
        depth = self.head.run(ops, x_d0, [r4, r3, r2, r1], clb, taps)
        return depth, [x_d0, r4, r3, r2, r1, out_conv]


class ExternalCoreBranchNet:

    def __init__(self, sd, prefix, bcfg, process_shape, dtype, device, provider):
        if provider is None:
            raise NotImplementedError(
                "branch type 'ZoeDepth' needs a relative-depth core: the MiDaS/BEiT encoder is an un-vendored torch.hub "
                "repository (midas.py:340).  Pass core_providers=(coarse, fine) to PatchFusion or call set_core_providers().")
        self.dtype, self.device, self.provider = dtype, device, provider
        self.C = branch_channels(bcfg)
        self.H, self.W = process_shape
        self.conv2 = pk.pack_conv(sd[prefix + "conv2.weight"], sd[prefix + "conv2.bias"], dtype=dtype).to(device)
        self.head = BinsHead(sd, prefix, self.C, bcfg, dtype, device, with_rel=True)

    def forward(self, ops, img, taps=None):
        dt, dev = self.dtype, self.device
        if hasattr(self.provider, "forward_nhwc"):
            if dt != F32:
                raise NotImplementedError("the native MiDaS core runs in float32 only (compute_dtype='fp32')")
            B, _, H, W = img.shape
            clb = self.head.new_clb_buffer(ops, B, H, W)
            _, feats = self.provider.forward_nhwc(ops, img, out_conv=clb[..., :32], rel=clb[..., 32 + self.head.emb:])
            btl, blocks = feats[0], feats[1:5]
            x_d0 = ops.empty(btl.shape[:3] + (self.C,), dt, dev)
            ops.conv(btl, self.conv2, x_d0)
            depth = self.head.run(ops, x_d0, blocks, clb, taps)
            return depth, [x_d0] + blocks + [clb[..., :32]]
        rel, feats = self.provider(img)
        assert len(feats) == 6, "provider must return [btlnck, x_block0..3, out_conv]"
        nhwc = [f.detach().to(dev).permute(0, 2, 3, 1).contiguous().to(dt) for f in feats]
        btl, blocks, outc = nhwc[0], nhwc[1:5], nhwc[5]
        B, H, W = rel.shape
        clb = self.head.new_clb_buffer(ops, B, H, W)
        ops.copy_channels(outc, clb[..., :32])
        tail = torch.zeros((B, H, W, 8), dtype=dt, device=dev)
        tail[..., 0] = rel.detach().to(device=dev, dtype=dt)
        clb[..., 32 + self.head.emb:] = tail
        x_d0 = ops.empty(btl.shape[:3] + (self.C,), dt, dev)
        ops.conv(btl, self.conv2, x_d0)
        depth = self.head.run(ops, x_d0, blocks, clb, taps)
        return depth, [x_d0] + blocks + [clb[..., :32]]


class G2LNet:
    DEPTH = [4, 4, 3, 3, 2, 2]
    HEADS = [32, 32, 16, 16, 8, 8]

    def __init__(self, sd, gcfg, dtype, device, prefix="guided_fusion."):
        self.dtype, self.device = dtype, device
        from .spec import GF_DEFAULT_IN_CHANNELS
        ch = list(gcfg.get("in_channels", GF_DEFAULT_IN_CHANNELS))[::-1]
        self.levels = []
        for i, C in enumerate(ch):
            g = f"{prefix}g2l_list.{i}."
            blocks = []
            for j in range(self.DEPTH[i]):
                b = f"{g}g2l_layer.blocks.{j}."

                def pc(name):
                    return pk.pack_conv(sd[b + name + ".weight"], sd[b + name + ".bias"], dtype=dtype).to(device)
                blocks.append(dict(n1=(_g(sd, b + "norm1.weight", device), _g(sd, b + "norm1.bias", device)),
                                   n2=(_g(sd, b + "norm2.weight", device), _g(sd, b + "norm2.bias", device)),
                                   qkv=pc("attn.qkv"), proj=pc("attn.proj"), fc1=pc("mlp.fc1"), fc2=pc("mlp.fc2"),
                                   bias_table=_g(sd, b + "attn.relative_position_bias_table", device),
                                   shift=0 if j % 2 == 0 else 6))
            self.levels.append(dict(C=C, heads=self.HEADS[i], blocks=blocks,
                                    ape=_g(sd, g + "absolute_pos_embed", device)[0],
                                    norm=(_g(sd, g + "g2l_layer_norm.weight", device), _g(sd, g + "g2l_layer_norm.bias", device))))

    def forward_level(self, ops, i, feat):
        dt, dev = self.dtype, self.device
        lv = self.levels[i]
        B, H, W, C = feat.shape
        Hp, Wp = int(math.ceil(H / 12)) * 12, int(math.ceil(W / 12)) * 12
        nt = B * Hp * Wp
        x = ops.empty((B, H, W, C), dt, dev)
# ... 126 lines not shown
```

patchfusion_amd/hip_ops.py:

```python
import ctypes as C

import torch

from . import _lib
from ._lib import ConvParams, check
from .packing import PackedConv, winograd_applies

_L = _lib.load()

ACT = {"none": 0, None: 0, "relu": 1, "gelu": 2, "softplus": 3}


def _stream():
    return C.c_void_p(torch.cuda.current_stream().cuda_stream)


def _p(t):
    if t is None:
        return None
    if not t.is_cuda:
        raise _lib.PfError("patchfusion_amd.hip_ops: tensor is not on the GPU (there is no CPU path)")
    if t.device.index != torch.cuda.current_device():
        raise _lib.PfError(f"patchfusion_amd.hip_ops: tensor lives on cuda:{t.device.index} but the current device is "
                           f"cuda:{torch.cuda.current_device()} (wrap the call in torch.cuda.device(...))")
# ... 280 lines not shown
                  "pf_conv_winograd_fused_timed")
            return ms.value
        HipOps._conv_exec(route, p, extra, x.device)
        e0, e1 = torch.cuda.Event(enable_timing=True), torch.cuda.Event(enable_timing=True)
        e0.record()
        for _ in range(int(_timed)):
            HipOps._conv_exec(route, p, extra, x.device)
        e1.record()
        e1.synchronize()
        return e0.elapsed_time(e1) / int(_timed)

    @staticmethod
    def gemm_planes_split3(V3, U3, Mw, T, cin, cout, iters=None):
        P = V3.shape[1]
        kmaj = V3.dim() == 5
        assert V3.dim() == U3.dim() and V3.dtype == U3.dtype == torch.bfloat16 and Mw.dtype == torch.float32 and U3.shape[:2] == (3, P)
        assert tuple(V3.shape) == ((3, P, cin // 32, T, 32) if kmaj else (3, P, T, cin)) and (U3.shape[2] * 32 if kmaj else U3.shape[3]) == cin
        assert V3.is_contiguous() and U3.is_contiguous() and Mw.is_contiguous() and Mw.numel() >= P * T * cout
        p = ConvParams()
        p.x, p.x_ld, p.B, p.H, p.W, p.Cin = V3.data_ptr(), cin, 1, 1, T, cin
        p.w, p.w_rows, p.Kpad = U3.data_ptr(), U3.shape[3] if kmaj else U3.shape[2], cin
        p.korder = 6 if kmaj else 0
        p.y, p.y_ld, p.OH, p.OW, p.Cout = Mw.data_ptr(), cout, 1, T, cout
        p.KH = p.KW = p.stride = 1
        p.act, p.shuffle, p.dtype, p.out_f32, p.batch = 0, 1, 1, 1, P
        p.x_bstride, p.w_bstride = V3.stride(0), U3.stride(0)
        for t in (V3, U3, Mw):
            _p(t)
        if iters is None:
            check(_L.pf_gemm_split3(C.byref(p), _stream()), "pf_gemm_split3")
            return Mw
        ms = C.c_float(0)
        check(_L.pf_gemm_split3_timed(C.byref(p), int(iters), C.byref(ms), _stream()), "pf_gemm_split3_timed")
        return ms.value

    @staticmethod
    def gemm_planes_split3_timed(V3, U3, Mw, T, cin, cout, iters):
        return HipOps.gemm_planes_split3(V3, U3, Mw, T, cin, cout, iters)

    @staticmethod
    def gemm_planes_timed(V, U, Mw, planes, T, cin, cout, iters):
        assert V.dtype == U.dtype == Mw.dtype == torch.float32 and V.numel() >= planes * T * cin and Mw.numel() >= planes * T * cout
        p = ConvParams()
        p.x, p.x_ld, p.B, p.H, p.W, p.Cin = V.data_ptr(), cin, 1, 1, T, cin
        p.w, p.w_rows, p.Kpad = U.data_ptr(), U.shape[1], U.shape[2]
        p.y, p.y_ld, p.OH, p.OW, p.Cout = Mw.data_ptr(), cout, 1, T, cout
        p.KH = p.KW = p.stride = 1
        p.shuffle, p.dtype = 1, 0
        p.batch, p.x_bstride, p.w_bstride, p.y_bstride = planes, T * cin, U.shape[1] * U.shape[2], T * cout
        for t in (V, U, Mw):
            _p(t)
        ms = C.c_float(0)
        check(_L.pf_conv_timed(C.byref(p), int(iters), C.byref(ms), _stream()), "pf_conv_timed")
        return ms.value

    @staticmethod
    def split3(x, y3):
        assert x.dtype == torch.float32 and y3.dtype == torch.bfloat16 and y3.dim() == 3 and y3.shape[0] == 3 and y3.is_contiguous()
        M, K = x.shape
        check(_L.pf_split3(_p(x), x.stride(0), _p(y3), y3.stride(1), y3.stride(0), M, K, _stream()), "pf_split3")
        return y3

    @staticmethod
    def _conv_split3_plan(x3, pw, y, act, res, res2):
        assert x3.dtype == torch.bfloat16 and x3.shape[0] == 3 and pw.w.dtype == torch.bfloat16
        split_out = y.dtype == torch.bfloat16
        p = ConvParams()
        korder = 0
        if x3.dim() == 4:
            assert x3.is_contiguous() and x3.shape[3] == 32 and x3.shape[1] * 32 == pw.cin
            M = x3.shape[2]
            p.x, p.x_ld = x3.data_ptr(), pw.cin
            korder |= 2
        else:
            assert x3.dim() == 3 and x3.stride(2) == 1 and x3.shape[2] >= pw.cin
            M = x3.shape[1]
            p.x, p.x_ld = x3.data_ptr(), x3.stride(1)
        p.B, p.H, p.W, p.Cin = 1, 1, M, pw.cin
        p.x_bstride = x3.stride(0)
        if pw.w.dim() == 4:
            assert pw.w.is_contiguous() and pw.w.shape[1] * 32 == pw.cin
            p.w, p.w_rows, p.Kpad, p.w_bstride = pw.w.data_ptr(), pw.w.shape[2], pw.cin, pw.w.stride(0)
            korder |= 4
        else:
            p.w, p.w_rows, p.Kpad, p.w_bstride = pw.w.data_ptr(), pw.w.shape[1], pw.w.shape[2], pw.w.stride(0)
        p.bias = pw.bias.data_ptr() if pw.bias is not None else None
        p.scale = pw.scale.data_ptr() if pw.scale is not None else None
        p.res = res.data_ptr() if res is not None else None
        p.res_ld = res.stride(-2) if res is not None else 0
        p.res2 = res2.data_ptr() if res2 is not None else None
        p.res2_ld = res2.stride(-2) if res2 is not None else 0
        if split_out and y.dim() == 4:
            assert y.is_contiguous() and tuple(y.shape) == (3, pw.cout // 32, M, 32) and pw.cout % 32 == 0
            p.y, p.y_ld, p.y_bstride, p.out_f32 = y.data_ptr(), pw.cout, y.stride(0), 0
            korder |= 8
        elif split_out:
            assert y.dim() == 3 and y.shape[0] == 3 and y.shape[1] == M and y.stride(2) == 1
            p.y, p.y_ld, p.y_bstride, p.out_f32 = y.data_ptr(), y.stride(1), y.stride(0), 0
        else:
            assert y.dtype == torch.float32 and y.stride(-1) == 1
            p.y, p.y_ld, p.out_f32 = y.data_ptr(), y.stride(-2), 1
        p.OH, p.OW, p.Cout = 1, M, pw.cout
        p.KH = p.KW = p.stride = 1
        p.act, p.shuffle, p.dtype, p.korder = ACT[act], 1, 1, korder
        for t in (x3, y, pw.w, res, res2):
            _p(t)
        for t in (res, res2):
            assert t is None or (t.dtype == torch.float32 and t.shape[-1] >= pw.cout and t.shape[-2] == M), "residuals are float32 [M, >= N]"
        assert y.dim() == 4 or (y.shape[-1] >= pw.cout and y.shape[-2] == M)
        return p

    @staticmethod
    def conv_split3(x3, pw: PackedConv, y, act=None, res=None, res2=None, _timed=None):
        key = (id(pw), x3.shape, x3.stride(), y.shape, y.stride(), y.dtype, act, x3.device,
               None if res is None else (res.shape, res.stride()), None if res2 is None else (res2.shape, res2.stride()))
        ent = _CONV_CACHE.get(key)
        if ent is None or ent[0] is not pw:
            if len(_CONV_CACHE) > 4096:
                _CONV_CACHE.clear()
            ent = (pw, HipOps._conv_split3_plan(x3, pw, y, act, res, res2))
            _CONV_CACHE[key] = ent
        else:
            p = ent[1]
            p.x, p.y = x3.data_ptr(), y.data_ptr()
            if res is not None:
                p.res = res.data_ptr()
            if res2 is not None:
                p.res2 = res2.data_ptr()
        p = ent[1]
        if _timed is not None:
            ms = C.c_float(0)
            check(_L.pf_gemm_split3_timed(C.byref(p), int(_timed), C.byref(ms), _stream()), "pf_gemm_split3_timed")
            return ms.value
        check(_L.pf_gemm_split3(C.byref(p), _stream()), "pf_gemm_split3")
        return y

    @staticmethod
    def _conv_f16x2_plan(x2, pw, y, act, res, res2, out_exp):
        assert x2.dtype == pw.w.dtype == torch.float16 and x2.dim() == 4 and x2.shape[0] == 2 and x2.shape[3] == 32 and x2.is_contiguous()
        assert x2.shape[1] * 32 == pw.cin and pw.w.dim() == 4 and pw.w.is_contiguous() and pw.col_exp is not None
        M = x2.shape[2]
        p = ConvParams()
        p.x, p.x_ld, p.x_bstride = x2.data_ptr(), pw.cin, x2.stride(0)
        p.B, p.H, p.W, p.Cin = 1, 1, M, pw.cin
        p.w, p.w_rows, p.Kpad, p.w_bstride = pw.w.data_ptr(), pw.w.shape[2], pw.cin, pw.w.stride(0)
        p.bias = pw.bias.data_ptr() if pw.bias is not None else None
        p.scale = pw.scale.data_ptr() if pw.scale is not None else None
        p.col_exp = _p(pw.col_exp)
        p.res = res.data_ptr() if res is not None else None
        p.res_ld = res.stride(-2) if res is not None else 0
        p.res2 = res2.data_ptr() if res2 is not None else None
        p.res2_ld = res2.stride(-2) if res2 is not None else 0
        korder = 6
        if y.dtype == torch.float16:
            assert y.is_contiguous() and tuple(y.shape) == (2, pw.cout // 32, M, 32) and pw.cout % 32 == 0
            assert out_exp is not None and out_exp.dtype == torch.int32 and out_exp.numel() >= pw.cout
            p.y, p.y_ld, p.y_bstride, p.out_f32, p.out_exp = y.data_ptr(), pw.cout, y.stride(0), 0, _p(out_exp)
            korder |= 16
        elif y.dtype == torch.bfloat16:
            assert y.dim() == 3 and y.shape[0] == 3 and y.shape[1] == M and y.stride(2) == 1 and y.shape[2] >= pw.cout
            p.y, p.y_ld, p.y_bstride, p.out_f32 = y.data_ptr(), y.stride(1), y.stride(0), 0
        else:
            assert y.dtype == torch.float32 and y.stride(-1) == 1 and y.shape[-2] == M and y.shape[-1] >= pw.cout
            p.y, p.y_ld, p.out_f32 = y.data_ptr(), y.stride(-2), 1
        p.OH, p.OW, p.Cout = 1, M, pw.cout
        p.KH = p.KW = p.stride = 1
        p.act, p.shuffle, p.dtype, p.korder = ACT[act], 1, 1, korder
        for t in (x2, y, pw.w, res, res2):
            _p(t)
        for t in (res, res2):
            assert t is None or (t.dtype == torch.float32 and t.shape[-1] >= pw.cout and t.shape[-2] == M), "residuals are float32 [M, >= N]"
        return p

    @staticmethod
    def conv_f16x2(x2, pw: PackedConv, y, act=None, res=None, res2=None, out_exp=None):
        key = ("f16x2", id(pw), x2.shape, y.shape, y.stride(), y.dtype, act, x2.device,
               None if res is None else (res.shape, res.stride()), None if res2 is None else (res2.shape, res2.stride()),
               None if out_exp is None else out_exp.data_ptr())
        ent = _CONV_CACHE.get(key)
        if ent is None or ent[0] is not pw:
            if len(_CONV_CACHE) > 4096:
                _CONV_CACHE.clear()
            ent = (pw, HipOps._conv_f16x2_plan(x2, pw, y, act, res, res2, out_exp))
            _CONV_CACHE[key] = ent
        else:
            p = ent[1]
            p.x, p.y = x2.data_ptr(), y.data_ptr()
            if res is not None:
                p.res = res.data_ptr()
            if res2 is not None:
                p.res2 = res2.data_ptr()
        check(_L.pf_gemm_f16x2(C.byref(ent[1]), _stream()), "pf_gemm_f16x2")
        return y

    @staticmethod
    def patch_im2col(img, out):
        B, _, H, W = img.shape
        assert img.dtype == torch.float32 and img.is_contiguous()
        check(_L.pf_patch_im2col(_p(img), B, H, W, _p(out), out.stride(0), _dt(out), _stream()), "pf_patch_im2col")

    @staticmethod
    def assemble_tokens(emb, tokens, cls, pos):
        B, S, D = tokens.shape
        assert emb.is_contiguous() and tokens.is_contiguous()
        check(_L.pf_assemble_tokens(_p(emb), _p(tokens), _p(cls), _p(pos), B, S, D, _dt(tokens), _stream()), "pf_assemble_tokens")

    @staticmethod
    def layernorm(x, y, g, b, eps, batches=1, in_rows_per_batch=None, in_row_offset=0, out_rows_per_batch=None):
        D = x.shape[-1]
        rows = x.numel() // D
        if in_rows_per_batch is None:
            in_rows_per_batch = out_rows_per_batch = rows
            batches = 1
        check(_L.pf_layernorm(_p(x), x.stride(-2), _p(y), y.stride(-2), _p(g), _p(b), float(eps), batches, in_rows_per_batch,
                              in_row_offset, out_rows_per_batch, D, _dt(x), _stream()), "pf_layernorm")

    @staticmethod
    def layernorm_split3(x, y3, g, b, eps):
        assert x.dtype == torch.float32 and y3.dtype == torch.bfloat16 and y3.shape[0] == 3
        M, D = x.shape
        if y3.dim() == 4:
            assert y3.is_contiguous() and tuple(y3.shape) == (3, D // 32, M, 32)
            check(_L.pf_layernorm_split3(_p(x), x.stride(0), _p(y3), D, y3.stride(0), 1, _p(g), _p(b), float(eps), M, D, _stream()),
                  "pf_layernorm_split3")
            return y3
        assert y3.dim() == 3 and y3.stride(2) == 1 and y3.shape[1] == M and y3.shape[2] == D
        check(_L.pf_layernorm_split3(_p(x), x.stride(0), _p(y3), y3.stride(1), y3.stride(0), 0, _p(g), _p(b), float(eps), M, D, _stream()),
              "pf_layernorm_split3")
        return y3

    @staticmethod
    def layernorm_f16x2(x, y2, g, b, eps, in_exp):
        assert x.dtype == torch.float32 and x.stride(-1) == 1 and y2.dtype == torch.float16 and in_exp.dtype == torch.int32
        M, D = x.shape
        assert y2.is_contiguous() and tuple(y2.shape) == (2, D // 32, M, 32) and in_exp.numel() == D
        check(_L.pf_layernorm_f16x2(_p(x), x.stride(0), _p(y2), _p(in_exp), _p(g), _p(b), float(eps), M, D, _stream()), "pf_layernorm_f16x2")
        return y2

    @staticmethod
    def vit_attention(qkv, out, B, S, heads):
        kmaj = int(out.dim() == 4)
        if qkv.dim() == 3:
            D = qkv.shape[2] // 3
            assert qkv.dtype == out.dtype == torch.bfloat16 and tuple(qkv.shape) == (3, B * S, 3 * D)
            assert tuple(out.shape) == ((3, D // 32, B * S, 32) if kmaj else (3, B * S, D))
            assert D == heads * 64 and qkv.is_contiguous() and out.is_contiguous()
            if _env("PF_ATTN_V2", "1") != "0":
                check(_L.pf_vit_attention_split3_v2(_p(qkv), qkv.stride(0), _p(out), out.stride(0), kmaj, B, S, heads, int(_env("PF_ATTN_QW", "0")),
                                                    int(_env("PF_ATTN_SCHED", "0")), _stream()), "pf_vit_attention_split3_v2")
                return
            check(_L.pf_vit_attention_split3(_p(qkv), qkv.stride(0), _p(out), out.stride(0), kmaj, B, S, heads, _stream()), "pf_vit_attention_split3")
            return
        D = qkv.shape[1] // 3
        assert D == heads * 64 and qkv.is_contiguous() and out.is_contiguous()
        if qkv.dtype == torch.float32 and out.dtype == torch.bfloat16:
            assert tuple(out.shape) == ((3, D // 32, B * S, 32) if kmaj else (3, B * S, D))
            check(_L.pf_vit_attention_qkv_split3(_p(qkv), _p(out), out.stride(0), kmaj, B, S, heads, _stream()), "pf_vit_attention_qkv_split3")
            return
        if qkv.dtype == torch.float32 and _env("PF_ATTN_QKV", "1") != "0":
            check(_L.pf_vit_attention_qkv(_p(qkv), _p(out), B, S, heads, 0, _stream()), "pf_vit_attention_qkv")
            return
        Sp = (S + 63) // 64 * 64
        q = torch.empty((B, heads, S, 64), dtype=qkv.dtype, device=qkv.device)
        k = torch.empty_like(q)
        vt = torch.empty((B, heads, 64, Sp), dtype=qkv.dtype, device=qkv.device)
        check(_L.pf_qkv_split(_p(qkv), B, S, heads, _p(q), _p(k), _p(vt), Sp, 0.125, _dt(qkv), _stream()), "pf_qkv_split")
        check(_L.pf_vit_attention(_p(q), _p(k), _p(vt), _p(out), B, S, Sp, heads, _dt(qkv), _stream()), "pf_vit_attention")

    @staticmethod
    def vit_attention_rpb(qkv, out, B, S, heads, tab, th, tw):
        kmaj = int(out.dim() == 4)
        D = heads * 64
        if qkv.dtype != torch.bfloat16 or tuple(qkv.shape) != (3, B * S, 3 * D) or not qkv.is_contiguous():
            raise ValueError(f"vit_attention_rpb: qkv must be contiguous bfloat16 [3, {B * S}, {3 * D}], got {qkv.dtype} {tuple(qkv.shape)}")
        if out.dtype != torch.bfloat16 or tuple(out.shape) != ((3, D // 32, B * S, 32) if kmaj else (3, B * S, D)) or not out.is_contiguous():
            raise ValueError(f"vit_attention_rpb: bad output planes {out.dtype} {tuple(out.shape)}")
        if S != th * tw + 1:
            raise ValueError(f"vit_attention_rpb: S = {S} is not th * tw + 1 = {th * tw + 1}")
        ntab = (2 * th - 1) * (2 * tw - 1) + 3
        if tab.dtype != torch.float32 or tuple(tab.shape) != (heads, ntab) or not tab.is_contiguous() or tab.device != qkv.device:
            raise ValueError(f"vit_attention_rpb: tab must be contiguous float32 [{heads}, {ntab}] on {qkv.device}")
        check(_L.pf_vit_attention_split3_rpb(_p(qkv), qkv.stride(0), _p(out), out.stride(0), kmaj, B, S, heads, _p(tab), th, tw,
                                             int(_env("PF_ATTN_QW", "0")), _stream()), "pf_vit_attention_split3_rpb")

    @staticmethod
    def patch_im2col_norm(img, out, patch, mean, std):
        B, Ci, H, W = img.shape
        if img.dtype != torch.float32 or not img.is_contiguous() or Ci != 3 or H % patch or W % patch:
            raise ValueError(f"patch_im2col_norm: img must be contiguous float32 [B,3,H,W] with H, W multiples of {patch}")
        if out.dtype != torch.float32 or out.dim() != 2 or out.shape[0] != B * (H // patch) * (W // patch) or out.shape[1] < 3 * patch * patch \
                or out.stride(1) != 1:
            raise ValueError(f"patch_im2col_norm: bad output {out.dtype} {tuple(out.shape)}")
        m3, s3 = (C.c_float * 3)(*[float(v) for v in mean]), (C.c_float * 3)(*[float(v) for v in std])
        check(_L.pf_patch_im2col_norm(_p(img), B, H, W, patch, C.cast(m3, C.c_void_p), C.cast(s3, C.c_void_p), _p(out), out.stride(0), _stream()),
              "pf_patch_im2col_norm")

    @staticmethod
    def readout_concat(x, y, B, S):
        D = x.shape[1]
        if x.dtype != torch.float32 or y.dtype != torch.float32 or x.shape[0] != B * S or x.stride(1) != 1 or y.stride(1) != 1:
            raise ValueError("readout_concat: float32 row-major operands required")
        if tuple(y.shape) != (B * (S - 1), 2 * D) or D % 4 or x.stride(0) % 4 or y.stride(0) % 4 or (x.data_ptr() | y.data_ptr()) & 15:
            raise ValueError(f"readout_concat: bad shapes / strides / alignment x {tuple(x.shape)} y {tuple(y.shape)}")
        check(_L.pf_readout_concat(_p(x), x.stride(0), B, S, D, _p(y), y.stride(0), _stream()), "pf_readout_concat")

    @staticmethod
    def swin_ln_partition(x, xw, g, b, eps, shift):
        B, H, W, Cc = x.shape
        assert xw.is_contiguous()
        check(_L.pf_swin_ln_partition(_p(x), _ld(x), _p(xw), _p(g), _p(b), float(eps), B, H, W, Cc, shift, _dt(x), _stream()),
              "pf_swin_ln_partition")

    @staticmethod
    def swin_window_attention(qkv, out, bias_table, B, Hp, Wp, Cc, heads, shift):
        assert qkv.is_contiguous() and out.is_contiguous() and bias_table.is_contiguous()
        check(_L.pf_swin_window_attention(_p(qkv), _p(out), _p(bias_table), B, Hp, Wp, Cc, heads, shift, _dt(qkv), _stream()),
              "pf_swin_window_attention")

    @staticmethod
    def swin_unpartition_add(proj, shortcut, y, shift):
        B, H, W, Cc = shortcut.shape
        check(_L.pf_swin_unpartition_add(_p(proj), _p(shortcut), _ld(shortcut), _p(y), _ld(y), B, H, W, Cc, shift, _dt(y), _stream()),
              "pf_swin_unpartition_add")

    @staticmethod
    def add_rowwise(x, pos):
        B, T, Cc = x.shape
        check(_L.pf_add_rowwise(_p(x), x.stride(1), _p(pos), B, T, Cc, _dt(x), _stream()), "pf_add_rowwise")

    @staticmethod
    def resize(x, y, add=None, dtype=None):
        x4, y4 = _as4(x), _as4(y)
        B, H, W, Cc = x4.shape
        _, OH, OW, _ = y4.shape
        cd = dtype if dtype is not None else (x4.dtype if x4.dtype != torch.float32 else y4.dtype)
        code = 1 if cd == torch.bfloat16 else 0
        in_f32 = int(x4.dtype == torch.float32)
        out_f32 = int(y4.dtype == torch.float32)
        if add is not None:
            assert add.dtype == y4.dtype
        check(_L.pf_resize_bilinear(_p(x4), _ld(x4), B, H, W, Cc, _p(y4), _ld(y4), OH, OW, _p(add), _ld(add) if add is not None else 0,
                                    in_f32, out_f32, code, _stream()), "pf_resize_bilinear")

    @staticmethod
    def resize_concat(xs, y):
        n = len(xs)
        y4 = _as4(y)
        B, OH, OW, Ct = y4.shape
        assert 2 <= n <= 3 and sum(x.shape[-1] for x in xs) <= Ct and all(x.dtype == y4.dtype and x.shape[0] == B for x in xs)
        ptrs = (C.c_void_p * n)(*[x.data_ptr() for x in xs])
        arr = lambda v: (C.c_int * n)(*v)
        for t in list(xs) + [y4]:
            _p(t)
        check(_L.pf_resize_concat(ptrs, arr([_ld(x) for x in xs]), arr([x.shape[1] for x in xs]), arr([x.shape[2] for x in xs]),
                                  arr([x.shape[3] for x in xs]), n, B, _p(y4), _ld(y4), OH, OW, _dt(y4), _stream()), "pf_resize_concat")

    @staticmethod
    def crop_resize(img, boxes, out):
        Cc, H, W = img.shape
        P, _, oh, ow = out.shape
        assert img.is_contiguous() and out.is_contiguous() and boxes.dtype == torch.int32
        check(_L.pf_crop_resize_planar(_p(img), Cc, H, W, _p(boxes), P, _p(out), oh, ow, _stream()), "pf_crop_resize_planar")

    @staticmethod
    def roi_align_depth(feat, rois, y, spatial_scale):
        Bf, _, H, W = feat.shape
        K, _, oh, ow = y.shape
        assert feat.is_contiguous() and y.is_contiguous() and feat.dtype == y.dtype == torch.float32
        check(_L.pf_roi_align(_p(feat), 1, Bf, H, W, 1, _p(rois), K, _p(y), 1, oh, ow, float(spatial_scale), 1, 1, 0, _stream()),
              "pf_roi_align")

    @staticmethod
    def roi_align(feat, rois, y, spatial_scale, dtype=None):
        Bf, H, W, Cc = feat.shape
        K, oh, ow, _ = y.shape
        code = 1 if (dtype or feat.dtype) == torch.bfloat16 else 0
        check(_L.pf_roi_align(_p(feat), _ld(feat), Bf, H, W, Cc, _p(rois), K, _p(y), _ld(y), oh, ow, float(spatial_scale),
                              int(feat.dtype == torch.float32), int(y.dtype == torch.float32), code, _stream()), "pf_roi_align")

    @staticmethod
    def maxpool2(x, y):
        B, H, W, Cc = x.shape
        check(_L.pf_maxpool2(_p(x), _ld(x), B, H, W, Cc, _p(y), _ld(y), _dt(x), _stream()), "pf_maxpool2")

    @staticmethod
    def copy_channels(x, y):
        x4, y4 = _as4(x), _as4(y)
        B, H, W, Cc = x4.shape
        code = 1 if torch.bfloat16 in (x4.dtype, y4.dtype) else 0
        check(_L.pf_copy_channels(_p(x4), _ld(x4), _p(y4), _ld(y4), B * H * W, Cc, int(x4.dtype == torch.float32),
                                  int(y4.dtype == torch.float32), code, _stream()), "pf_copy_channels")

    @staticmethod
    def pack_fusion_input(cdepth, fdepth, crops, y):
        B, h, w, c8 = y.shape
        assert c8 == 8 and y.is_contiguous() and cdepth.is_contiguous() and fdepth.is_contiguous() and crops.is_contiguous()
        check(_L.pf_pack_fusion_input(_p(cdepth), _p(fdepth), _p(crops), _p(y), B, h, w, _dt(y), _stream()), "pf_pack_fusion_input")

    @staticmethod
    def copy_plane(src, dst):
        dst.copy_(src[:, 0], non_blocking=True)

    @staticmethod
    def nhwc_to_nchw(x, Cc=None):
        B, H, W, Ct = x.shape
        Cc = Cc or Ct
        y = torch.empty((B, Cc, H, W), dtype=torch.float32, device=x.device)
        code = 1 if x.dtype == torch.bfloat16 else 0
        check(_L.pf_nhwc_to_nchw_f32(_p(x), _ld(x), _p(y), B, H, W, Cc, int(x.dtype == torch.float32), code, _stream()), "pf_nhwc_to_nchw_f32")
        return y

    @staticmethod
    def attractor(A, n_attr, b_prev, out, a_stride=1, a_eps=0.0, attractor_type="inv", kind="mean"):
        B, h, w, nb = out.shape
        _, hp, wp, _ = b_prev.shape
        assert A.dtype == b_prev.dtype == out.dtype == torch.float32 and b_prev.is_contiguous() and out.is_contiguous()
        assert A.shape[-1] >= (n_attr - 1) * a_stride + 1 and kind in ("mean", "sum")
        check(_L.pf_attractor(_p(A), _ld(A), n_attr, int(a_stride), float(a_eps), int(attractor_type == "exp"), int(kind == "sum"),
                              _p(b_prev), hp, wp, _p(out), B, h, w, nb, _stream()), "pf_attractor")

    @staticmethod
    def seed_bin_centers(x, out, min_depth, max_depth, bounded, normalize):
# ... 120 lines not shown
```

patchfusion_amd/packing.py:

```python
import math
from dataclasses import dataclass
from typing import Optional

import torch


def round_up(x, m):
    return (x + m - 1) // m * m


@dataclass
class PackedConv:
    w: torch.Tensor
    bias: Optional[torch.Tensor]
    scale: Optional[torch.Tensor]
    KH: int
    KW: int
    cin: int
    cout: int
    cout_real: int
    shuffle: int = 1
    korder: int = 0
    wino_m: int = 0
    wino_u: Optional[torch.Tensor] = None
# ... 110 lines not shown
        b = (beta - mean * f) if b is None else (b - mean) * f + beta
    if cin_map is None:
        cin_map = [(0, cin, 0)]
    if cin_total is None:
        cin_total = round_up(max(d + n for _, n, d in cin_map), 8)
    assert cin_total % 8 == 0
    cout_store = round_up(cout, 4)
    rows = round_up(cout_store, 16)
    wk = torch.zeros(rows, KH, KW, cin_total)
    for s0, n, d0 in cin_map:
        wk[:cout, :, :, d0:d0 + n] = w[:, s0:s0 + n].permute(0, 2, 3, 1)
    K = KH * KW * cin_total
    Kpad = round_up(K, k_chunk(dtype))
    wp = torch.zeros(rows, Kpad)
    korder = 1 if (dtype == torch.float32 and KH * KW > 1 and cin_total % 32 == 0) else 0
    if korder:
        wp[:, :K] = wk.reshape(rows, KH * KW, cin_total // 32, 32).permute(0, 2, 1, 3).reshape(rows, K)
    else:
        wp[:, :K] = wk.reshape(rows, K)
    bp = None
    if b is not None:
        bp = torch.zeros(rows)
        bp[:cout] = b
    sp = None
    if scale is not None:
        sp = torch.zeros(rows)
        sp[:cout] = scale.detach().float().cpu()
    wm = winograd_mode() if (scale is None and winograd_eligible(cout_store, cin_total, KH, KW, dtype)) else 0
    wu = winograd_filters(wk, wm) if wm else None
    wup = winograd_filters_fused(wk) if wm == 4 else None
    wu3 = (torch.stack(split3(wu)).view(3, wu.shape[0], wu.shape[1], wu.shape[2] // 32, 32).permute(0, 1, 3, 2, 4).contiguous()
           if (wm == 4 and winograd_split3_enabled()) else None)
    if wm == 0 and scale is None and winograd_fused_only_eligible(cout_store, cin_total, KH, KW, dtype):
        wm, wup = 4, winograd_filters_fused(wk)
    w3 = (rows_to_kmajor(torch.stack(split3(wk.reshape(rows, cin_total))).contiguous())
          if (dtype == torch.float32 and KH == 1 and KW == 1 and cin_total % 32 == 0 and conv1x1_split3_enabled()) else None)
    return PackedConv(wp.to(dtype).contiguous(), bp, sp, KH, KW, cin_total, cout_store, cout, korder=korder, wino_m=wm, wino_u=wu, wino_up=wup, wino_u3=wu3,
                      w3=w3)


def conv1x1_split3_enabled():
    import os
    return os.environ.get("PF_CONV1X1_SPLIT3", "1") != "0"


def split3(x):
    x = x.float()
    h = x.to(torch.bfloat16)
    r = x - h.float()
    m = r.to(torch.bfloat16)
    l = (r - m.float()).to(torch.bfloat16)
    return h, m, l


def split3_kmajor_enabled():
    import os
    return os.environ.get("PF_SPLIT3_KMAJOR", "1") != "0"


def rows_to_kmajor(t):
    *lead, rows, K = t.shape
    assert K % 32 == 0
    n = len(lead)
    return t.reshape(*lead, rows, K // 32, 32).permute(*range(n), n + 1, n, n + 2).contiguous()


def kmajor_to_rows(t):
    *lead, nk, rows, c = t.shape
    n = len(lead)
    return t.permute(*range(n), n + 1, n, n + 2).reshape(*lead, rows, nk * c)


def pack_conv_split3(weight, bias=None, *, scale=None, kmajor=None):
    w = weight.detach().float().cpu()
    if w.dim() == 4:
        assert w.shape[2] == 1 and w.shape[3] == 1
        w = w[:, :, 0, 0]
    cout, cin = w.shape
    assert cin % 32 == 0, "split GEMM: K must be a multiple of 32"
    cout_store = round_up(cout, 4)
    rows = round_up(cout_store, 16)
    wp = torch.zeros(rows, cin)
    wp[:cout] = w
    planes = torch.stack(split3(wp)).contiguous()
    if split3_kmajor_enabled() if kmajor is None else kmajor:
        planes = rows_to_kmajor(planes)
    bp = None
    if bias is not None:
        bp = torch.zeros(rows)
        bp[:cout] = bias.detach().float().cpu()
    sp = None
    if scale is not None:
        sp = torch.zeros(rows)
        sp[:cout] = scale.detach().float().cpu()
    return PackedConv(planes, bp, sp, 1, 1, cin, cout_store, cout)



def layernorm_bound(gamma, beta):
    g, b = gamma.detach().double().cpu(), beta.detach().double().cpu()
    return g.abs() * math.sqrt(g.numel() - 1) + b.abs()


def gelu_linear_bound(weight, bias, in_bound):
    w = weight.detach().double().cpu()
    z = w.abs() @ in_bound.double()
    if bias is not None:
        z = z + bias.detach().double().cpu().abs()
    return torch.clamp(z, min=0.17)


def _clog2(a):
    f, e = math.frexp(a)
    return e - 1 if f == 0.5 else e


def bound_exponents(bound):
    return torch.tensor([_clog2(float(b)) - 14 if b > 0 else 0 for b in bound.double().tolist()], dtype=torch.int32)


def split_f16x2(v):
    v = v.float()
    h = v.half()
    return h, (v - h.float()).half()


def pack_conv_f16x2(weight, bias=None, scale=None, in_bound=None):
    w = weight.detach().float().cpu()
    cout, cin = w.shape
    assert cin % 32 == 0, "fp16x2 GEMM: K must be a multiple of 32"
    assert in_bound is not None and in_bound.numel() == cin
    cout_store = round_up(cout, 4)
    rows = round_up(cout_store, 16)
    e = bound_exponents(in_bound)
    wp = torch.zeros(rows, cin)
    wp[:cout] = w
    mant, ex = torch.frexp(wp.double().abs())
    cl = torch.where(mant == 0.5, ex - 1, ex).long() + e.long()[None, :]
    cl = torch.where(wp != 0, cl, torch.full_like(cl, -(1 << 30)))
    f = cl.max(dim=1).values
    f = torch.where(f > -(1 << 30), f - 15, torch.zeros_like(f))
    v = torch.ldexp(wp.double(), (e.long()[None, :] - f[:, None]).double())
    planes = rows_to_kmajor(torch.stack(split_f16x2(v.float())).contiguous())
    bp = sp = None
    if bias is not None:
        bp = torch.zeros(rows)
        bp[:cout] = bias.detach().float().cpu()
    if scale is not None:
        sp = torch.zeros(rows)
        sp[:cout] = scale.detach().float().cpu()
    return PackedConv(planes, bp, sp, 1, 1, cin, cout_store, cout, col_exp=f.to(torch.int32), in_exp=e)


def pack_conv_transpose(weight, bias, *, dtype):
    w = weight.detach().float().cpu()
    cin, cout, s, s2 = w.shape
    assert s == s2 and cout % 4 == 0 and cin % 8 == 0
    rows_real = s * s * cout
    rows = round_up(rows_real, 16)
    Kpad = round_up(cin, k_chunk(dtype))
    wp = torch.zeros(rows, Kpad)
    wp[:rows_real, :cin] = w.permute(2, 3, 1, 0).reshape(rows_real, cin)
    bp = torch.zeros(round_up(cout, 16))
    bp[:cout] = bias.detach().float().cpu()
    return PackedConv(wp.to(dtype).contiguous(), bp, None, 1, 1, cin, rows_real, rows_real, shuffle=s)


def unpack_conv(pc: PackedConv):
    K = pc.KH * pc.KW * pc.cin
    w = pc.w.float()[:pc.cout, :K]
    if pc.korder:
        w = w.reshape(pc.cout, pc.cin // 32, pc.KH * pc.KW, 32).permute(0, 2, 1, 3)
    return w.reshape(pc.cout, pc.KH, pc.KW, pc.cin).permute(0, 3, 1, 2).contiguous()


@dataclass
class BinsTail:
    w0f: torch.Tensor
    b0: torch.Tensor
    w2: torch.Tensor
    b2: torch.Tensor
    nq: int
    rel_off: int
    mlp0: PackedConv
    mlp2: PackedConv

    def to(self, device):
        self.w0f, self.b0, self.w2, self.b2 = (t.to(device) for t in (self.w0f, self.b0, self.w2, self.b2))
        return self


def bins_tail_weights(mlp0: PackedConv, mlp2: PackedConv, emb: int):
    if mlp0.w.dtype != torch.float32 or mlp0.KH != 1 or mlp2.KH != 1 or emb != 128 or mlp0.cout_real != 80 or mlp2.cout_real != 4:
        return None
    if mlp0.cin not in (160, 168) or mlp2.cin != 80 or mlp0.bias is None or mlp2.bias is None or mlp0.scale is not None or mlp2.scale is not None:
        return None
    W0 = unpack_conv(mlp0).cpu()[:80, :, 0, 0]
    ctot = W0.shape[1]
    nq = (ctot + 15) // 16
    Wp = torch.zeros(80, nq * 16)
    Wp[:, :ctot] = W0
    w0f = Wp.view(5, 16, nq, 4, 4).permute(2, 0, 3, 1, 4).reshape(nq, 5, 64, 4).contiguous()
    W2 = unpack_conv(mlp2).cpu()[:4, :80, 0, 0].contiguous()
    return BinsTail(w0f, mlp0.bias.cpu()[:80].clone().float(), W2, mlp2.bias.cpu()[:4].clone().float(), nq, 160, mlp0, mlp2)


def vit_pos_embed(pos_embed, th, tw):
    import torch.nn.functional as F
    pos = pos_embed.detach().float().cpu()
    n = pos.shape[1] - 1
    g = int(math.sqrt(n))
    if th * tw == n and th == tw:
        return pos[0].contiguous()
    dim = pos.shape[-1]
    grid = pos[:, 1:].reshape(1, g, g, dim).permute(0, 3, 1, 2)
    grid = F.interpolate(grid, scale_factor=(float(th + 0.1) / g, float(tw + 0.1) / g), mode="bicubic", antialias=False)
    assert grid.shape[-2] == th and grid.shape[-1] == tw
    grid = grid.permute(0, 2, 3, 1).reshape(-1, dim)
    return torch.cat([pos[0, :1], grid], dim=0).contiguous()


def beit_rel_pos_table(table, pretrain, th, tw):
    import math

    import torch.nn.functional as F
    t = table.detach().float().cpu()
    old = 2 * pretrain - 1
    assert t.dim() == 2 and t.shape[0] == old * old + 3, tuple(t.shape)
    sub = t[:old * old].reshape(1, old, old, -1).permute(0, 3, 1, 2)
    new = F.interpolate(sub, size=(2 * th - 1, 2 * tw - 1), mode="bilinear")
    new = new.permute(0, 2, 3, 1).reshape((2 * th - 1) * (2 * tw - 1), -1)
    full = torch.cat([new, t[old * old:]])
    return (full * math.log2(math.e)).t().contiguous()
```

Baseline: 101.2 patches/s.

## Add f16x2 split-precision ViT attention kernel with per-head exponent scaling

Adds a new ViT attention kernel that consumes QKV as two fp16 planes (hi/lo split) with per-channel exponent scaling derived from weight and LayerNorm bounds. It uses 32x32x16 f16 MFMA, LDS DMA pipelining and a key-split path for short tail query blocks. The QKV GEMM now writes f16x2 directly, and optionally the projection also runs in f16x2, replacing the bf16x3 split path. This is meant to cut the MFMA passes and the memory traffic of the three-plane bf16 emulation, at the cost of precision that rests on static bound analysis.

```diff
diff --git a/include/pf_hip.h b/include/pf_hip.h
--- a/include/pf_hip.h
+++ b/include/pf_hip.h
@@ -70,6 +70,8 @@
 int pf_vit_attention_split3(const void* qkv3, long plane_in, void* out3, long plane_out, int kmajor, int B, int S, int Hh, void* stream);
 int pf_vit_attention_split3_v2(const void* qkv3, long plane_in, void* out3, long plane_out, int kmajor, int B, int S, int Hh, int queries_per_wave,
                                int schedule, void* stream);
+int pf_vit_attention_f16x2(const void* qkv2, long plane_in, const int* qk_exp, void* out, long plane_out, const int* v_exp3, int B, int S, int Hh,
+                           void* stream);
 int pf_vit_attention_split3_rpb(const void* qkv3, long plane_in, void* out3, long plane_out, int kmajor, int B, int S, int Hh, const float* tab,
                                 int th, int tw, int queries_per_wave, void* stream);
 int pf_split3(const float* x, int x_ld, void* y, int y_ld, long plane, long rows, int cols, void* stream);
diff --git a/patchfusion_amd/_lib.py b/patchfusion_amd/_lib.py
--- a/patchfusion_amd/_lib.py
+++ b/patchfusion_amd/_lib.py
@@ -61,6 +61,7 @@
     "pf_vit_attention_qkv_split3": [vp, vp, cl, ci, ci, ci, ci, vp],
     "pf_vit_attention_split3": [vp, cl, vp, cl, ci, ci, ci, ci, vp],
     "pf_vit_attention_split3_v2": [vp, cl, vp, cl, ci, ci, ci, ci, ci, ci, vp],
+    "pf_vit_attention_f16x2": [vp, cl, vp, vp, cl, vp, ci, ci, ci, vp],
     "pf_vit_attention_split3_rpb": [vp, cl, vp, cl, ci, ci, ci, ci, vp, ci, ci, ci, vp],
     "pf_patch_im2col_norm": [vp, ci, ci, ci, ci, vp, vp, vp, ci, vp],
     "pf_readout_concat": [vp, ci, ci, ci, ci, vp, ci, vp],
diff --git a/patchfusion_amd/csrc/attn_split3.hip b/patchfusion_amd/csrc/attn_split3.hip
--- a/patchfusion_amd/csrc/attn_split3.hip
+++ b/patchfusion_amd/csrc/attn_split3.hip
@@ -1,6 +1,7 @@
 #include "pf_common.h"
 #include "../../include/pf_hip.h"
 
+#include <atomic>
 #include <cstdlib>
 #include <type_traits>
 
@@ -724,6 +725,386 @@
 #endif
 }
 
+typedef __attribute__((ext_vector_type(2))) _Float16 f16x2_t;
+constexpr int HB_BYTES = 2 * 32 * 128;
+constexpr int PIPE_H_LDS = 6 * HB_BYTES;
+constexpr float PSHIFT_H = 12.0f, RESCALE_H = 15.0f;
+
+__device__ __forceinline__ uint32_t cvt_pk_h(float lo, float hi) {
+  return __builtin_bit_cast(uint32_t, __builtin_convertvector((f32x2_t){lo, hi}, f16x2_t));
+}
+__device__ __forceinline__ f16x8 tr_pair_h(const char* p0, const char* p1) {
+  const v4s a = __builtin_amdgcn_ds_read_tr16_b64_v4i16((lds_v4s*)p0);
+  const v4s b = __builtin_amdgcn_ds_read_tr16_b64_v4i16((lds_v4s*)p1);
+  return __builtin_bit_cast(f16x8, __builtin_shufflevector(a, b, 0, 1, 2, 3, 4, 5, 6, 7));
+}
+
+__global__ __launch_bounds__(256, 2) void vit_attention_f16x2_pipe_kernel(const uint16_t* __restrict__ qkv2, long plane_in, const int* __restrict__ qk_exp,
+                                                                          uint16_t* __restrict__ out2, long plane_out, const int* __restrict__ v_exp3, int S,
+                                                                          int Hh, float qscale0, long kmaj_rows, int n_qb, int BH) {
+  extern __shared__ __attribute__((aligned(16))) char smem[];
+  char* const Kr = smem;
+  char* const Vr = smem + 3 * HB_BYTES;
+  const int tid = threadIdx.x, lane = tid & 63;
+  const int wave = __builtin_amdgcn_readfirstlane(tid >> 6);
+  const int c = lane & 31, hi = lane >> 5;
+  int bh, qb;
+  {
+    const int bid = (int)blockIdx.x;
+    const bool tail = (S & 127) != 0 && (BH & 7) == 0 && n_qb > 1;
+    if (tail) {
+      if (bid < BH) { bh = bid; qb = n_qb - 1; }
+      else {
+        const int l = bid - BH, idx = l >> 3, nf = n_qb - 1;
+        bh = (idx / nf) * 8 + (l & 7);
+        qb = idx % nf;
+      }
+    } else {
+      const int l = xcd_remap(bid, (int)gridDim.x);
+      bh = l / n_qb;
+      qb = l - bh * n_qb;
+    }
+  }
+  const int b = bh / Hh, h = bh - b * Hh;
+  const int NB = (S + 31) / 32;
+  const bool ksplit = S - qb * 128 <= 32 && NB >= 8;
+  const int q0 = qb * 128 + (ksplit ? 0 : wave * 32);
+  const bool has_q = q0 < S;
+  const int D = Hh * 64;
+  const long rs = 3L * D;
+  const uint16_t* base = qkv2 + (long)b * S * rs + h * 64;
+  const float qscale = ldexpf(qscale0, qk_exp[h]);
+
+  const unsigned rs_b = (unsigned)(rs * 2);
+  const unsigned kchunk = (unsigned)(((lane & 7) ^ ((lane >> 4) & 3)) << 4);
+  const unsigned vchunk = (unsigned)(((lane & 7) ^ (((lane >> 4) & 1) << 2)) << 4);
+  const unsigned kr_lds = lds_addr_of(Kr), vr_lds = lds_addr_of(Vr);
+  auto issue = [&](int jb, int which, unsigned lds_dst) {
+    const char* sb = reinterpret_cast<const char*>(base + which * D);
+    const unsigned chunk = which == 1 ? kchunk : vchunk;
+    if (jb * 32 + 32 <= S) {
+      const unsigned lane_off = (unsigned)(jb * 32 + (lane >> 3)) * rs_b;
+#pragma unroll
+      for (int i = 0; i < 2; ++i) {
+        const int p = wave * 2 + i;
+        const unsigned ch = which == 1 ? chunk ^ (unsigned)((p & 1) << 6) : chunk;
+        dma16(sb + (long)(p >> 2) * plane_in * 2, lane_off + ch + (unsigned)((p & 3) * 8) * rs_b, lds_dst + p * 1024);
+      }
+    } else {
+#pragma unroll
+      for (int i = 0; i < 2; ++i) {
+        const int p = wave * 2 + i;
+        const unsigned ch = which == 1 ? chunk ^ (unsigned)((p & 1) << 6) : chunk;
+        const int row = min(jb * 32 + (p & 3) * 8 + (lane >> 3), S - 1);
+        dma16(sb + (long)(p >> 2) * plane_in * 2, ch + (unsigned)row * rs_b, lds_dst + p * 1024);
+      }
+    }
+  };
+  issue(0, 1, kr_lds);
+  issue(1, 1, kr_lds + HB_BYTES);
+  issue(2, 1, kr_lds + 2 * HB_BYTES);
+  issue(0, 2, vr_lds);
+
+  uint4 qf[2][4];
+  {
+    const int qi = min(q0 + c, S - 1);
+#pragma unroll
+    for (int pl = 0; pl < 2; ++pl)
+#pragma unroll
+      for (int ks = 0; ks < 4; ++ks) qf[pl][ks] = *reinterpret_cast<const uint4*>(base + pl * plane_in + (long)qi * rs + 16 * ks + 8 * hi);
+  }
+  f32x16 o[2];
+#pragma unroll
+  for (int t = 0; t < 2; ++t)
+#pragma unroll
+    for (int i = 0; i < 16; ++i) o[t][i] = 0.f;
+  float m_run = -INFINITY, l_run = 0.f, a_pend = 1.f;
+  f32x16 sA, sB;
+  uint4 pA[2][2], pB[2][2];
+#pragma unroll
+  for (int pl = 0; pl < 2; ++pl)
+#pragma unroll
+    for (int i = 0; i < 2; ++i) pA[pl][i] = pB[pl][i] = make_uint4(0, 0, 0, 0);
+
+  const char* kbase[4];
+#pragma unroll
+  for (int ks = 0; ks < 4; ++ks) kbase[ks] = Kr + c * 128 + (((2 * ks + hi) ^ ((c >> 1) & 7)) << 4);
+  const int j16 = lane & 15, jb1 = (j16 >> 3) & 1;
+  const char* vbase[2];
+#pragma unroll
+  for (int t = 0; t < 2; ++t) vbase[t] = Vr + (4 * hi + (j16 >> 2)) * 128 + ((2 * (t ^ jb1) + (c >> 4)) << 5) + ((j16 & 3) << 3);
+
+  __builtin_amdgcn_s_waitcnt(0x0070);
+  barrier_lds();
+
+  auto step = [&](auto qk_c, auto sm_c, auto mask_c, auto pv_c, auto par_c, int ks_off, int vs_off, int rem) {
+    constexpr bool QK = decltype(qk_c)::value, SM = decltype(sm_c)::value, MASK = decltype(mask_c)::value, PV = decltype(pv_c)::value;
+    constexpr int PAR = decltype(par_c)::value;
+    f32x16& s_next = PAR ? sA : sB;
+    f32x16& s_cur = PAR ? sB : sA;
+    uint4 (&p_cur)[2][2] = PAR ? pB : pA;
+    uint4 (&p_prev)[2][2] = PAR ? pA : pB;
+    if (!has_q) return;
+    uint4 kfs[2][2];
+    f16x8 vfs[2][2];
+    float pv[16];
+    float m_new = 0.f;
+    auto load_group = [&](auto n_c) {
+      constexpr int n = decltype(n_c)::value;
+      if constexpr (QK) {
+#pragma unroll
+        for (int pl = 0; pl < 2; ++pl) kfs[n & 1][pl] = *reinterpret_cast<const uint4*>(kbase[n] + ks_off + pl * 4096);
+      }
+      if constexpr (PV) {
+#pragma unroll
+        for (int pl = 0; pl < 2; ++pl) {
+          const char* p = vbase[n & 1] + vs_off + pl * 4096 + (n >> 1) * 2048;
+          vfs[n & 1][pl] = tr_pair_h(p, p + 1024);
+        }
+      }
+    };
+    auto mfma_slot = [&](auto n_c, auto i_c) {
+      constexpr int n = decltype(n_c)::value, i = decltype(i_c)::value;
+      constexpr int term = (QK && PV) ? (i >> 1) : i;
+      constexpr bool on_s = QK && (!PV || (i & 1) == 0);
+      constexpr int PA = term == 1 ? 1 : 0;
+      constexpr int PB_ = term == 0 ? 1 : 0;
+      if constexpr (on_s) {
+        if constexpr (n == 0 && term == 0)
+          s_next = __builtin_amdgcn_mfma_f32_32x32x16_f16(__builtin_bit_cast(f16x8, kfs[n & 1][PA]), __builtin_bit_cast(f16x8, qf[PB_][n]),
+                                                          f32x16{0.f, 0.f, 0.f, 0.f, 0.f, 0.f, 0.f, 0.f, 0.f, 0.f, 0.f, 0.f, 0.f, 0.f, 0.f, 0.f}, 0, 0, 0);
+        else
+          s_next = __builtin_amdgcn_mfma_f32_32x32x16_f16(__builtin_bit_cast(f16x8, kfs[n & 1][PA]), __builtin_bit_cast(f16x8, qf[PB_][n]), s_next, 0, 0, 0);
+      } else {
+        o[n & 1] = __builtin_amdgcn_mfma_f32_32x32x16_f16(vfs[n & 1][PA], __builtin_bit_cast(f16x8, p_prev[PB_][n >> 1]), o[n & 1], 0, 0, 0);
+      }
+    };
+    auto sm_head = [&]() {
+      if (MASK) {
+#pragma unroll
+        for (int i = 0; i < 16; ++i)
+          if ((i & 3) + 8 * (i >> 2) + 4 * hi >= rem) s_cur[i] = -INFINITY;
+      }
+      const float t0 = max3f(s_cur[0], s_cur[1], s_cur[2]), t1 = max3f(s_cur[3], s_cur[4], s_cur[5]), t2 = max3f(s_cur[6], s_cur[7], s_cur[8]);
+      const float t3 = max3f(s_cur[9], s_cur[10], s_cur[11]), t4 = max3f(s_cur[12], s_cur[13], s_cur[14]);
+      const float u0 = max3f(t0, t1, t2), u1 = max3f(t3, t4, s_cur[15]);
+      float mx = max3f(u0, u1, u1);
+      const auto y = __builtin_amdgcn_permlane32_swap(__float_as_uint(mx), __float_as_uint(mx), false, false);
+      mx = max3f(__uint_as_float(y[0]), __uint_as_float(y[1]), __uint_as_float(y[1]));
+      const float mb = mx * qscale;
+      const bool need = mb > m_run + RESCALE_H;
+      m_new = need ? mb - PSHIFT_H : m_run;
+      a_pend = need ? __builtin_amdgcn_exp2f(m_run - m_new) : 1.0f;
+      m_run = m_new;
+    };
+    float psum = 0.f, ra[8], rb[8];
+    auto sm_exp1 = [&](int i) {
+      pv[i] = __builtin_amdgcn_exp2f(fmaf(s_cur[i], qscale, -m_new));
+      psum += pv[i];
+    };
+    auto sm_split_a = [&](int u) {
+#pragma clang fp contract(off)
+      const uint32_t hw = cvt_pk_h(pv[2 * u], pv[2 * u + 1]);
+      const f16x2_t hv = __builtin_bit_cast(f16x2_t, hw);
+      ra[u] = pv[2 * u] - (float)hv[0];
+      rb[u] = pv[2 * u + 1] - (float)hv[1];
+      (&p_cur[0][u >> 2].x)[u & 3] = hw;
+    };
+    auto sm_split_b = [&](int u) { (&p_cur[1][u >> 2].x)[u & 3] = cvt_pk_h(ra[u], rb[u]); };
+    constexpr int NSLOT = (QK ? 3 : 0) + (PV ? 3 : 0);
+    auto valu_chunk = [&](auto n_c, auto i_c) {
+      constexpr int n = decltype(n_c)::value, i = decltype(i_c)::value;
+      if constexpr (SM) {
+        if constexpr (NSLOT == 6) {
+          if constexpr (n == 0) {
+            sm_exp1(2 * i); sm_exp1(2 * i + 1);
+            if constexpr (i < 2) { sm_exp1(12 + 2 * i); sm_exp1(13 + 2 * i); }
+            if constexpr (i == 5) l_run = l_run * a_pend + psum;
+          } else {
+            constexpr int gs = 6 * (n - 1) + i;
+            if constexpr (gs < 16) {
+              if constexpr ((gs & 1) == 0) sm_split_a(gs / 2);
+              else sm_split_b(gs / 2);
+            }
+          }
+        } else if constexpr (NSLOT == 3) {
+          if constexpr (n == 0) {
+#pragma unroll
+            for (int e = 0; e < 5; ++e) sm_exp1(5 * i + e);
+            if constexpr (i == 2) { sm_exp1(15); l_run = l_run * a_pend + psum; }
+          } else {
+            constexpr int gs = 3 * (n - 1) + i;
+            if constexpr (gs < 8) { sm_split_a(gs); sm_split_b(gs); }
+          }
+        }
+      }
+    };
+    if constexpr (PV) {
+      const float a_use = a_pend;
+      if (__builtin_amdgcn_ballot_w64(a_use != 1.0f) != 0) {
+#pragma unroll
+        for (int t = 0; t < 2; ++t)
+#pragma unroll
+          for (int i = 0; i < 16; ++i) o[t][i] *= a_use;
+      }
+    }
+    if constexpr (QK || PV) load_group(std::integral_constant<int, 0>{});
+    if constexpr (SM) sm_head();
+    __builtin_amdgcn_sched_barrier(0);
+    auto slot = [&](auto n_c, auto i_c) {
+      constexpr int i = decltype(i_c)::value;
+      if constexpr (i < NSLOT) {
+        mfma_slot(n_c, i_c);
+        valu_chunk(n_c, i_c);
+        __builtin_amdgcn_sched_barrier(0);
+      }
+    };
+    auto group = [&](auto n_c) {
+      constexpr int n = decltype(n_c)::value;
+      if constexpr (NSLOT > 0) {
+        if constexpr (n < 3) {
+          load_group(std::integral_constant<int, n + 1>{});
+          __builtin_amdgcn_sched_barrier(0);
+        }
+        slot(n_c, std::integral_constant<int, 0>{});
+        slot(n_c, std::integral_constant<int, 1>{});
+        slot(n_c, std::integral_constant<int, 2>{});
+        slot(n_c, std::integral_constant<int, 3>{});
+        slot(n_c, std::integral_constant<int, 4>{});
+        slot(n_c, std::integral_constant<int, 5>{});
+      }
+    };
+    group(std::integral_constant<int, 0>{});
+    group(std::integral_constant<int, 1>{});
+    group(std::integral_constant<int, 2>{});
+    group(std::integral_constant<int, 3>{});
+    if constexpr (NSLOT == 0 && SM) {
+#pragma unroll
+      for (int i = 0; i < 16; ++i) sm_exp1(i);
+      l_run = l_run * a_pend + psum;
+#pragma unroll
+      for (int u = 0; u < 8; ++u) { sm_split_a(u); sm_split_b(u); }
+    }
+  };
+  auto turn = [&](int j, int ks, int vs) {
+    asm volatile("s_waitcnt vmcnt(4) lgkmcnt(0)\n\ts_barrier" ::: "memory");
+    issue(j + 4, 1, kr_lds + ks);
+    issue(j + 2, 2, vr_lds + vs);
+  };
+  using T = std::true_type;
+  using F = std::false_type;
+  using P0 = std::integral_constant<int, 0>;
+  using P1 = std::integral_constant<int, 1>;
+  constexpr int HB = HB_BYTES;
+  if (!ksplit) {
+    step(T{}, F{}, F{}, F{}, P1{}, 0, 0, 0);
+    turn(-1, 0, HB);
+    if (NB > 1) step(T{}, T{}, F{}, F{}, P0{}, HB, 0, 0);
+    else step(F{}, T{}, T{}, F{}, P0{}, 0, 0, S);
+    turn(0, HB, 2 * HB);
+    int ks = 2 * HB, vs = 0;
+    int j = 1;
+    for (; j + 1 <= NB - 2; j += 2) {
+      step(T{}, T{}, F{}, T{}, P1{}, ks, vs, 0);
+      turn(j, ks, vs);
+      ks = ks == 2 * HB ? 0 : ks + HB;
+      vs = vs == 2 * HB ? 0 : vs + HB;
+      step(T{}, T{}, F{}, T{}, P0{}, ks, vs, 0);
+      turn(j + 1, ks, vs);
+      ks = ks == 2 * HB ? 0 : ks + HB;
+      vs = vs == 2 * HB ? 0 : vs + HB;
+    }
+    if (j <= NB - 2) {
+      step(T{}, T{}, F{}, T{}, P1{}, ks, vs, 0);
+      turn(j, ks, vs);
+      ks = ks == 2 * HB ? 0 : ks + HB;
+      vs = vs == 2 * HB ? 0 : vs + HB;
+      ++j;
+    }
+    const int rem = S - (NB - 1) * 32;
+    if (NB > 1) {
+      if (j & 1) step(F{}, T{}, T{}, T{}, P1{}, ks, vs, rem);
+      else step(F{}, T{}, T{}, T{}, P0{}, ks, vs, rem);
+      vs = vs == 2 * HB ? 0 : vs + HB;
+      ++j;
+    }
+    barrier_all();
+    if (j & 1) step(F{}, F{}, F{}, T{}, P1{}, 0, vs, 0);
+    else step(F{}, F{}, F{}, T{}, P0{}, 0, vs, 0);
+  } else {
+    const int remk = S - (NB - 1) * 32;
+    int ksj = 0, vsj = HB;
+    for (int jj = -1; jj <= NB; ++jj) {
+      if (((jj + 1 - wave) & 3) == 0 && jj + 1 < NB) step(T{}, F{}, F{}, F{}, P1{}, ksj, vsj, 0);
+      else if (((jj - wave) & 3) == 0 && jj >= 0 && jj < NB) {
+        if (jj == NB - 1) step(F{}, T{}, T{}, F{}, P0{}, ksj, vsj, remk);
+        else step(F{}, T{}, F{}, F{}, P0{}, ksj, vsj, 0);
+      } else if (((jj - 1 - wave) & 3) == 0 && jj >= 1 && jj - 1 < NB) step(F{}, F{}, F{}, T{}, P1{}, ksj, vsj, 0);
+      if (jj <= NB - 2) turn(jj, ksj, vsj);
+      else if (jj == NB - 1) barrier_all();
+      ksj = ksj == 2 * HB ? 0 : ksj + HB;
+      vsj = vsj == 2 * HB ? 0 : vsj + HB;
+    }
+    __syncthreads();
+    float* park = reinterpret_cast<float*>(smem);
+    if (wave > 0) {
+      float* pw = park + (wave - 1) * 34 * 64 + lane;
+      pw[0] = m_run;
+      pw[64] = l_run;
+#pragma unroll
+      for (int t = 0; t < 2; ++t)
+#pragma unroll
+        for (int i = 0; i < 16; ++i) pw[(2 + t * 16 + i) * 64] = o[t][i];
+    }
+    __syncthreads();
+    if (wave > 0) return;
+#pragma unroll 1
+    for (int w = 0; w < 3; ++w) {
+      const float* pw = park + w * 34 * 64 + lane;
+      const float mw = pw[0], lw = pw[64];
+      const float mn = fmaxf(m_run, mw);
+      const float f0 = __builtin_amdgcn_exp2f(m_run - mn), fw = __builtin_amdgcn_exp2f(mw - mn);
+      l_run = l_run * f0 + lw * fw;
+#pragma unroll
+      for (int t = 0; t < 2; ++t)
+#pragma unroll
+        for (int i = 0; i < 16; ++i) o[t][i] = o[t][i] * f0 + pw[(2 + t * 16 + i) * 64] * fw;
+      m_run = mn;
+    }
+  }
+
+  if (!has_q) return;
+  float l = l_run;
+  {
+    const auto y = __builtin_amdgcn_permlane32_swap(__float_as_uint(l), __float_as_uint(l), false, false);
+    l = __uint_as_float(y[0]) + __uint_as_float(y[1]);
+  }
+  const float inv = 1.0f / l;
+  const int qo = q0 + c;
+  if (qo < S) {
+#pragma unroll
+    for (int t = 0; t < 2; ++t)
+#pragma unroll
+      for (int rq = 0; rq < 4; ++rq) {
+#pragma clang fp contract(off)
+        const int col = h * 64 + 32 * t + 8 * rq + 4 * hi;
+        const float w0 = o[t][4 * rq] * inv, w1 = o[t][4 * rq + 1] * inv, w2 = o[t][4 * rq + 2] * inv, w3 = o[t][4 * rq + 3] * inv;
+        if (v_exp3) {
+          const int4 e = *reinterpret_cast<const int4*>(v_exp3 + col);
+          const float w4[4] = {ldexpf(w0, e.x), ldexpf(w1, e.y), ldexpf(w2, e.z), ldexpf(w3, e.w)};
+          store_split3(out2 + split3_at((long)b * S + qo, col, D, kmaj_rows), plane_out, w4);
+          continue;
+        }
+        const uint32_t h0 = cvt_pk_h(w0, w1), h1 = cvt_pk_h(w2, w3);
+        const f16x2_t a = __builtin_bit_cast(f16x2_t, h0), bb = __builtin_bit_cast(f16x2_t, h1);
+        const uint32_t l0 = cvt_pk_h(w0 - (float)a[0], w1 - (float)a[1]), l1 = cvt_pk_h(w2 - (float)bb[0], w3 - (float)bb[1]);
+        uint16_t* dst = out2 + split3_at((long)b * S + qo, col, D, kmaj_rows);
+        *reinterpret_cast<uint2*>(dst) = make_uint2(h0, h1);
+        *reinterpret_cast<uint2*>(dst + plane_out) = make_uint2(l0, l1);
+      }
+  }
+}
+
 constexpr int V2_LDS = 3 * KS_BYTES;
 
 }
@@ -740,13 +1121,20 @@
   if (const char* e = getenv("PF_ATTN_DBG")) dbg = atoi(e);
   if (const char* e = getenv("PF_ATTN_LDS")) lds2 = ldsp = atoi(e);
 #endif
-  static int attr_done = 0;
-  if (attr_done != lds2) {
+  static std::atomic<unsigned long long> attr_done{0};
+#ifdef PF_ATTN_DBG
+  static std::atomic<int> attr_lds{0};
+  if (attr_lds.exchange(lds2) != lds2) attr_done.store(0, std::memory_order_release);
+#endif
+  int dev = 0;
+  hipGetDevice(&dev);
+  const unsigned long long dev_bit = 1ull << (dev & 63);
+  if (!(attr_done.load(std::memory_order_acquire) & dev_bit)) {
     const void* ks[3] = {reinterpret_cast<const void*>(vit_attention_split3_v2_kernel<1>), reinterpret_cast<const void*>(vit_attention_split3_v2_kernel<2>),
                          reinterpret_cast<const void*>(vit_attention_split3_pipe_kernel)};
     for (int i = 0; i < 3; ++i)
       if (hipFuncSetAttribute(ks[i], hipFuncAttributeMaxDynamicSharedMemorySize, i < 2 ? lds2 : ldsp) != hipSuccess) return PF_ERR_LAUNCH;
-    attr_done = lds2;
+    attr_done.fetch_or(dev_bit, std::memory_order_release);
   }
   int qw = queries_per_wave;
   if (schedule != 1) qw = 32;
@@ -768,6 +1156,27 @@
   return hipGetLastError() == hipSuccess ? PF_OK : PF_ERR_LAUNCH;
 }
 
+extern "C" int pf_vit_attention_f16x2(const void* qkv2, long plane_in, const int* qk_exp, void* out, long plane_out, const int* v_exp3, int B, int S, int Hh,
+                                      void* stream) {
+  void* out2 = out;
+  if (!qkv2 || !qk_exp || !out2 || B <= 0 || S <= 0 || Hh <= 0 || plane_in < (long)B * S * Hh * 192 || plane_out < (long)B * S * Hh * 64) return PF_ERR_ARG;
+  if ((long)S * Hh * 192 * 2 >= (1L << 31)) return PF_ERR_ARG;
+  static std::atomic<unsigned long long> attr_done{0};
+  int dev = 0;
+  hipGetDevice(&dev);
+  const unsigned long long dev_bit = 1ull << (dev & 63);
+  if (!(attr_done.load(std::memory_order_acquire) & dev_bit)) {
+    if (hipFuncSetAttribute(reinterpret_cast<const void*>(vit_attention_f16x2_pipe_kernel), hipFuncAttributeMaxDynamicSharedMemorySize, PIPE_H_LDS) != hipSuccess)
+      return PF_ERR_LAUNCH;
+    attr_done.fetch_or(dev_bit, std::memory_order_release);
+  }
+  const float qscale = 0.125f * 1.4426950408889634f;
+  const int n_qb = (S + 127) / 128;
+  hipLaunchKernelGGL(vit_attention_f16x2_pipe_kernel, dim3(n_qb * B * Hh), dim3(256), PIPE_H_LDS, reinterpret_cast<hipStream_t>(stream),
+                     (const uint16_t*)qkv2, plane_in, qk_exp, (uint16_t*)out2, plane_out, v_exp3, S, Hh, qscale, (long)B * S, n_qb, B * Hh);
+  return hipGetLastError() == hipSuccess ? PF_OK : PF_ERR_LAUNCH;
+}
+
 extern "C" int pf_vit_attention_split3_rpb(const void* qkv3, long plane_in, void* out3, long plane_out, int kmajor, int B, int S, int Hh,
                                            const float* tab, int th, int tw, int queries_per_wave, void* stream) {
   if (!qkv3 || !out3 || !tab || B <= 0 || Hh <= 0 || th <= 0 || tw <= 0 || plane_in < (long)B * S * Hh * 192 || plane_out < (long)B * S * Hh * 64)
diff --git a/patchfusion_amd/csrc/gemm_split3.hip b/patchfusion_amd/csrc/gemm_split3.hip
--- a/patchfusion_amd/csrc/gemm_split3.hip
+++ b/patchfusion_amd/csrc/gemm_split3.hip
@@ -692,7 +692,7 @@
         if (nok) fexp = *reinterpret_cast<const int4*>(reinterpret_cast<const int*>(p.scale) + (long)e_z * p.w_rows + n);
       } else if constexpr (F16) {
         if (nok) fexp = *reinterpret_cast<const int4*>(p.col_exp + n);
-        if (nok && (p.korder & 16)) oexp = *reinterpret_cast<const int4*>(p.out_exp + n);
+        if (nok && (p.korder & 48)) oexp = *reinterpret_cast<const int4*>(p.out_exp + n);
       }
       if constexpr (!BARE) {
         if (nok) {
@@ -770,6 +770,22 @@
               const auto s0 = __builtin_amdgcn_permlane16_swap(hw[0], lw2[0], false, false);
               const auto s1 = __builtin_amdgcn_permlane16_swap(hw[1], lw2[1], false, false);
               if (ok) *reinterpret_cast<uint4*>(reinterpret_cast<uint16_t*>(p.y) + split3_at(m, ne, p.y_ld, M) + (oddg ? p.y_bstride : 0)) = make_uint4(s0[0], s1[0], s0[1], s1[1]);
+            } else if (F16 && (p.korder & 32)) {
+              const int oe[4] = {oexp.x, oexp.y, oexp.z, oexp.w};
+              uint32_t hw[2], lw2[2];
+#pragma unroll
+              for (int r = 0; r < 4; r += 2) {
+                const float t0 = ldexpf(v[h][r], -oe[r]), t1 = ldexpf(v[h][r + 1], -oe[r + 1]);
+                const _Float16 h0 = (_Float16)t0, h1 = (_Float16)t1;
+                const _Float16 l0 = (_Float16)(t0 - (float)h0), l1 = (_Float16)(t1 - (float)h1);
+                hw[r >> 1] = (uint32_t)__builtin_bit_cast(uint16_t, h0) | ((uint32_t)__builtin_bit_cast(uint16_t, h1) << 16);
+                lw2[r >> 1] = (uint32_t)__builtin_bit_cast(uint16_t, l0) | ((uint32_t)__builtin_bit_cast(uint16_t, l1) << 16);
+              }
+              if (ok) {
+                uint16_t* yp = reinterpret_cast<uint16_t*>(p.y) + (long)m * p.y_ld + n;
+                *reinterpret_cast<uint2*>(yp) = make_uint2(hw[0], hw[1]);
+                *reinterpret_cast<uint2*>(yp + p.y_bstride) = make_uint2(lw2[0], lw2[1]);
+              }
             } else if (F16 || !(p.korder & 8)) {
               if (ok) store_split3(reinterpret_cast<bf16_t*>(p.y) + split3_at(m, n, p.y_ld, 0), p.y_bstride, v[h]);
             } else {
@@ -1174,15 +1190,17 @@
 extern "C" int pf_gemm_f16x2(const pf_conv_params* p, void* stream) {
   if (!p || !p->x || !p->w || !p->y || !p->col_exp) return PF_ERR_ARG;
   const long M = (long)p->B * p->OH * p->OW;
-  if (p->KH != 1 || p->KW != 1 || p->stride != 1 || p->pad != 0 || p->shuffle > 1 || p->batch > 1 || (p->korder & ~16) != 6) return PF_ERR_ARG;
+  if (p->KH != 1 || p->KW != 1 || p->stride != 1 || p->pad != 0 || p->shuffle > 1 || p->batch > 1 || (p->korder & ~48) != 6 || (p->korder & 48) == 48)
+    return PF_ERR_ARG;
   if (p->Cin <= 0 || p->Cin % 32 || p->x_ld != p->Cin || p->Kpad != p->Cin || p->Cout <= 0 || p->Cout % 4 || p->y_ld % 4 || p->w_rows < p->Cout ||
       p->w_rows % 4)
     return PF_ERR_ARG;
   if (M <= 0 || M * 64 >= (1L << 31) || (long)p->w_rows * 64 >= (1L << 31) || p->x_bstride <= 0 || p->w_bstride <= 0) return PF_ERR_ARG;
   if ((p->res && p->res_ld % 4) || (p->res2 && p->res2_ld % 4)) return PF_ERR_ARG;
-  if (p->out_f32 && (p->korder & 16)) return PF_ERR_ARG;
+  if (p->out_f32 && (p->korder & 48)) return PF_ERR_ARG;
   if (!p->out_f32 && p->y_bstride <= 0) return PF_ERR_ARG;
   if ((p->korder & 16) && (!p->out_exp || p->y_ld != p->Cout || p->Cout % 32)) return PF_ERR_ARG;
+  if ((p->korder & 32) && (!p->out_exp || p->y_ld < p->Cout || p->y_bstride % 4 || (reinterpret_cast<size_t>(p->y) & 7))) return PF_ERR_ARG;
   return launch_persist192_f16_linear(*p, reinterpret_cast<hipStream_t>(stream));
 }
 
diff --git a/patchfusion_amd/engine.py b/patchfusion_amd/engine.py
--- a/patchfusion_amd/engine.py
+++ b/patchfusion_amd/engine.py
@@ -18,6 +18,12 @@
     import os
     v = os.environ.get("PF_VIT_F16X2", "1")
     return v == "2" or (v != "0" and crops)
+
+
+def vit_attn_f16x2_enabled():
+    import os
+    v = os.environ.get("PF_VIT_ATTN_F16X2", "1")
+    return 0 if v == "0" else 2 if v == "2" else 1
 
 
 def attention_split3_enabled():
@@ -162,6 +168,9 @@
                     return pk.pack_conv_split3(sd[name + ".weight"], sd[name + ".bias"] if bias else None, **kw).to(dev)
                 return _pc(name, bias, **kw)
         self.f16x2 = self.split3 and vit_f16x2_enabled(crops) and getattr(ops, "conv_f16x2", None) is not None
+        self.attn_f16x2 = (self.f16x2 and crops and vit_attn_f16x2_enabled() != 0 and attention_split3_enabled() and pk.split3_kmajor_enabled()
+                           and getattr(ops, "vit_attention_f16x2", None) is not None)
+        self.proj_f16x2 = self.attn_f16x2 and vit_attn_f16x2_enabled() == 2
         self.blocks = []
         for i in range(self.depth):
             b = f"{v}blocks.{i}."
@@ -175,10 +184,21 @@
                                          pk.gelu_linear_bound(w1, b1, bn2)).to(dev)
             else:
                 qkv, fc1, fc2 = pc(b + "attn.qkv"), pc(b + "mlp.fc1"), pc(b + "mlp.fc2", scale=sd[b + "ls2.gamma"])
+            attn = None
+            if self.attn_f16x2:
+                attn = pk.vit_attn_f16x2_scales(sd[b + "attn.qkv.weight"], sd[b + "attn.qkv.bias"], bn1, self.heads)
+                if self.proj_f16x2:
+                    proj = pk.pack_conv_f16x2(sd[b + "attn.proj.weight"], sd[b + "attn.proj.bias"], sd[b + "ls1.gamma"], attn.v_bound).to(dev)
+                else:
+                    proj = pc(b + "attn.proj", scale=sd[b + "ls1.gamma"])
+                attn = attn.to(dev)
+            else:
+                proj = pc(b + "attn.proj", scale=sd[b + "ls1.gamma"])
             self.blocks.append(dict(
                 n1=(_g(sd, b + "norm1.weight", dev), _g(sd, b + "norm1.bias", dev)),
                 qkv=qkv,
-                proj=pc(b + "attn.proj", scale=sd[b + "ls1.gamma"]),
+                attn=attn,
+                proj=proj,
                 n2=(_g(sd, b + "norm2.weight", dev), _g(sd, b + "norm2.bias", dev)),
                 fc1=fc1,
                 fc2=fc2))
@@ -243,6 +263,10 @@
             qkv = ops.empty((3, B * S, 3 * D), torch.bfloat16, dev) if attention_split3_enabled() else ops.empty((B * S, 3 * D), dt, dev)
             if self.f16x2:
                 hbuf, mid = (ops.empty((2, n // 32, B * S, 32), torch.float16, dev) for n in (D, 4 * D))
+            if self.attn_f16x2:
+                qkv = ops.empty((2, B * S, 3 * D), torch.float16, dev)
+                if self.proj_f16x2:
+                    att = ops.empty((2, D // 32, B * S, 32), torch.float16, dev)
         else:
             hbuf = ops.empty((B * S, D), dt, dev)
             qkv = ops.empty((B * S, 3 * D), dt, dev)
@@ -251,9 +275,18 @@
         for i, blk in enumerate(self.blocks):
             if self.f16x2:
                 ops.layernorm_f16x2(x, hbuf, blk["n1"][0], blk["n1"][1], 1e-6, blk["qkv"].in_exp)
-                ops.conv_f16x2(hbuf, blk["qkv"], qkv)
-                ops.vit_attention(qkv, att, B, S, self.heads)
-                ops.conv_split3(att, blk["proj"], x, res=x)
+                if self.attn_f16x2:
+                    ops.conv_f16x2(hbuf, blk["qkv"], qkv, out_exp=blk["attn"].out_exp)
+                    if self.proj_f16x2:
+                        ops.vit_attention_f16x2(qkv, att, B, S, self.heads, blk["attn"].qk_exp)
+                        ops.conv_f16x2(att, blk["proj"], x, res=x)
+                    else:
+                        ops.vit_attention_f16x2(qkv, att, B, S, self.heads, blk["attn"].qk_exp, v_exp=blk["attn"].v_exp)
+                        ops.conv_split3(att, blk["proj"], x, res=x)
+                else:
+                    ops.conv_f16x2(hbuf, blk["qkv"], qkv)
+                    ops.vit_attention(qkv, att, B, S, self.heads)
+                    ops.conv_split3(att, blk["proj"], x, res=x)
                 ops.layernorm_f16x2(x, hbuf, blk["n2"][0], blk["n2"][1], 1e-6, blk["fc1"].in_exp)
                 ops.conv_f16x2(hbuf, blk["fc1"], mid, act="gelu", out_exp=blk["fc2"].in_exp)
                 ops.conv_f16x2(mid, blk["fc2"], x, res=x)
diff --git a/patchfusion_amd/hip_ops.py b/patchfusion_amd/hip_ops.py
--- a/patchfusion_amd/hip_ops.py
+++ b/patchfusion_amd/hip_ops.py
@@ -456,7 +456,12 @@
         p.res2 = res2.data_ptr() if res2 is not None else None
         p.res2_ld = res2.stride(-2) if res2 is not None else 0
         korder = 6
-        if y.dtype == torch.float16:
+        if y.dtype == torch.float16 and y.dim() == 3:
+            assert y.shape[0] == 2 and y.shape[1] == M and y.stride(2) == 1 and y.shape[2] >= pw.cout and y.stride(1) % 4 == 0
+            assert out_exp is not None and out_exp.dtype == torch.int32 and out_exp.numel() >= pw.cout
+            p.y, p.y_ld, p.y_bstride, p.out_f32, p.out_exp = y.data_ptr(), y.stride(1), y.stride(0), 0, _p(out_exp)
+            korder |= 32
+        elif y.dtype == torch.float16:
             assert y.is_contiguous() and tuple(y.shape) == (2, pw.cout // 32, M, 32) and pw.cout % 32 == 0
             assert out_exp is not None and out_exp.dtype == torch.int32 and out_exp.numel() >= pw.cout
             p.y, p.y_ld, p.y_bstride, p.out_f32, p.out_exp = y.data_ptr(), pw.cout, y.stride(0), 0, _p(out_exp)
@@ -572,6 +577,23 @@
         check(_L.pf_vit_attention(_p(q), _p(k), _p(vt), _p(out), B, S, Sp, heads, _dt(qkv), _stream()), "pf_vit_attention")
 
     @staticmethod
+    def vit_attention_f16x2(qkv2, out2, B, S, heads, qk_exp, v_exp=None):
+        D = heads * 64
+        if v_exp is not None:
+            if out2.dtype != torch.bfloat16 or tuple(out2.shape) != (3, D // 32, B * S, 32) or not out2.is_contiguous():
+                raise ValueError(f"vit_attention_f16x2: bad bf16x3 output planes {out2.dtype} {tuple(out2.shape)}")
+            if v_exp.dtype != torch.int32 or v_exp.numel() != D or not v_exp.is_contiguous() or v_exp.device != qkv2.device:
+                raise ValueError(f"vit_attention_f16x2: v_exp must be contiguous int32 [{D}] on {qkv2.device}")
+        if qkv2.dtype != torch.float16 or tuple(qkv2.shape) != (2, B * S, 3 * D) or not qkv2.is_contiguous():
+            raise ValueError(f"vit_attention_f16x2: qkv2 must be contiguous float16 [2, {B * S}, {3 * D}], got {qkv2.dtype} {tuple(qkv2.shape)}")
+        if v_exp is None and (out2.dtype != torch.float16 or tuple(out2.shape) != (2, D // 32, B * S, 32) or not out2.is_contiguous()):
+            raise ValueError(f"vit_attention_f16x2: bad output planes {out2.dtype} {tuple(out2.shape)}")
+        if qk_exp.dtype != torch.int32 or qk_exp.numel() != heads or not qk_exp.is_contiguous() or qk_exp.device != qkv2.device:
+            raise ValueError(f"vit_attention_f16x2: qk_exp must be contiguous int32 [{heads}] on {qkv2.device}")
+        check(_L.pf_vit_attention_f16x2(_p(qkv2), qkv2.stride(0), _p(qk_exp), _p(out2), out2.stride(0), None if v_exp is None else _p(v_exp), B, S, heads,
+                                        _stream()), "pf_vit_attention_f16x2")
+
+    @staticmethod
     def vit_attention_rpb(qkv, out, B, S, heads, tab, th, tw):
         kmaj = int(out.dim() == 4)
         D = heads * 64
diff --git a/patchfusion_amd/packing.py b/patchfusion_amd/packing.py
--- a/patchfusion_amd/packing.py
+++ b/patchfusion_amd/packing.py
@@ -286,6 +286,39 @@
     return PackedConv(planes, bp, sp, 1, 1, cin, cout_store, cout, col_exp=f.to(torch.int32), in_exp=e)
 
 
+def linear_bound(weight, bias, in_bound):
+    z = weight.detach().double().cpu().abs() @ in_bound.double()
+    if bias is not None:
+        z = z + bias.detach().double().cpu().abs()
+    return z
+
+
+@dataclass
+class AttnF16x2Scales:
+    out_exp: torch.Tensor
+    qk_exp: torch.Tensor
+    v_bound: torch.Tensor
+    v_exp: Optional[torch.Tensor] = None
+
+    def to(self, device):
+        self.out_exp, self.qk_exp = self.out_exp.to(device), self.qk_exp.to(device)
+        self.v_exp = self.out_exp[2 * self.v_bound.numel():]
+        return self
+
+
+def vit_attn_f16x2_scales(qkv_weight, qkv_bias, ln_bound, heads):
+    bound = linear_bound(qkv_weight, qkv_bias, ln_bound)
+    D = bound.numel() // 3
+    assert bound.numel() == 3 * D and D == heads * 64
+    r = bound_exponents(bound).long()
+    rq, rk = r[:D].reshape(heads, 64), r[D:2 * D].reshape(heads, 64)
+    E = (rq + rk).max(dim=1).values
+    eq = rq + (E[:, None] - rq - rk) // 2
+    ek = E[:, None] - eq
+    out_exp = torch.cat([eq.reshape(-1), ek.reshape(-1), r[2 * D:]]).to(torch.int32).contiguous()
+    return AttnF16x2Scales(out_exp, E.to(torch.int32).contiguous(), bound[2 * D:].clone(), out_exp[2 * D:])
+
+
 def pack_conv_transpose(weight, bias, *, dtype):
     w = weight.detach().float().cpu()
     cin, cout, s, s2 = w.shape
```

Measured after the change: 103.0 patches/s, median of 6. 1.02x the previous value.
